# Thieso/BoundPlanner

Hardware: AMD Instinct MI355X
Metric: MPC solves/sec (whole node), iiwa14 7-DOF, N=20 (higher is better)
Workload: dtype f64; 1 GPU; BASELINE configs[2]: 8192-batch, randomized convex-set obstacles, N=20, cold start, tol 1e-5, max_iter 100; a fresh batch every step; batch_per_gpu=8192, horizon=20, distinct_batches=22, fresh_batches=16, hess=2, solver_handles_in_flight=4, batches_in_flight=44, pool_slots=16384

## Files before the change

__graft_entry__.py:

```python
import os
import subprocess
import sys

ROOT = os.path.dirname(os.path.abspath(__file__))
CSRC = os.path.join(ROOT, "boundplanner_amd", "csrc")
HIP_LIB = os.path.join(CSRC, "libboundmpc_hip.so")
_COMMON = ["bmpc_platform_hip.hpp", "bmpc_device.hpp", "bmpc_internal.hpp"]
_HANDLE = ["bmpc_handle.hpp", "bmpc_pipeline.hpp", "bmpc_stage.hpp", "bmpc_robot.hpp", "../../include/boundmpc.h"]
HIP_OBJS = {
    "bmpc_fk.o": ("bmpc_fk.hip", [], _COMMON),
    "bmpc_pipeline.o": ("bmpc_pipeline.hip", [], _COMMON + ["bmpc_pipeline.hpp", "bmpc_pair_kernels.hpp", "bmpc_ric_kernel.hpp",
                                                            "bmpc_stage.hpp", "bmpc_stage_matrix.hpp"]),
    "bmpc_loop.o": ("bmpc_loop.hip", [], _COMMON + ["bmpc_loop.hpp", "bmpc_freespace.hpp", "bmpc_robot.hpp", "../../include/boundmpc.h"]),
    "bmpc_capi.o": ("bmpc_capi.hip", [], _COMMON + _HANDLE + ["bmpc_staging.hpp"]),
    "bmpc_capi_batch.o": ("bmpc_capi_batch.hip", [], _COMMON + _HANDLE + ["bmpc_staging.hpp", "bmpc_ik.hpp", "bmpc_sets.hpp",
                                                                          "bmpc_freespace.hpp"]),
    "bmpc_ik.o": ("bmpc_ik.hip", [], _COMMON + ["bmpc_ik.hpp"]),
    "bmpc_sets.o": ("bmpc_sets.hip", [], _COMMON + ["bmpc_sets.hpp", "bmpc_freespace.hpp"]),
}


def _stale(target, deps):
    if not os.path.exists(target):
        return True
    t = os.path.getmtime(target)
    return any(os.path.getmtime(d) > t for d in deps if os.path.exists(d))


def build():
    flags = ["--offload-arch=gfx950", "-O3", "-std=c++17", "-fPIC", "-ffp-contract=on"]
    objs, relink = [], not os.path.exists(HIP_LIB)
    for obj, (src, defs, hdrs) in HIP_OBJS.items():
        o = os.path.join(CSRC, obj)
        if _stale(o, [os.path.join(CSRC, f) for f in [src] + hdrs]):
            subprocess.check_call(["hipcc", *flags, *defs, "-c", os.path.join(CSRC, src), "-o", o])
        objs.append(o)
    if relink or _stale(HIP_LIB, objs):
        subprocess.check_call(["hipcc", "--offload-arch=gfx950", "-shared", "-fPIC", "-o", HIP_LIB, *objs])
    subprocess.check_call(["make", "-C", os.path.join(ROOT, "oracle")], stdout=subprocess.DEVNULL)
    sys.path.insert(0, ROOT)
    import boundplanner_amd
    from boundplanner_amd import solver
    lib = solver.load_library()
    for name in solver.EXPORTS:
        getattr(lib, name)


def smoke():
    sys.path.insert(0, ROOT)
    sys.path.insert(0, os.path.join(ROOT, "tests"))
    import numpy as np
    import oracle_lib as O
    from boundplanner_amd import scenes
    from boundplanner_amd.solver import HipBoundMPC
    N, B = 10, 8
    be = HipBoundMPC(N)
    batch = scenes.make_batch(B, N, 1024, be.fk)
    r = be.solve_batch(batch["x0"], batch["lbx"], batch["ubx"], batch["p"])
    ro = O.solve_batch(N, batch["x0"], batch["lbx"], batch["ubx"], batch["p"])
    assert (r["status"] == 0).all(), r["status"]
    err = np.abs(r["x"][:, 28 * N:40 * N] - ro["x"][:, 28 * N:40 * N]).max()
    assert err < 2e-5, err
    print(f"smoke ok: B={B} N={N} iters={r['iters'].tolist()} max|pv_hip - pv_oracle|={err:.2e} kernel {be.last_kernel_ms():.2f} ms")


if __name__ == "__main__":
    build()
    if len(sys.argv) > 1 and sys.argv[1] == "smoke":
        smoke()
```

boundplanner_amd/csrc/bmpc_internal.hpp:

```cpp
#pragma once
#include <hip/hip_runtime.h>

#include <cstddef>
#include <cstdlib>

struct bmpc_handle;
namespace bmpc {
struct RobotConst;
struct IkOpts;
struct SetScene;
template <int DEV> struct PipeArgsT;
typedef PipeArgsT<0> PipeArgsH;
}

inline int env_int(const char* name, int dflt) { const char* e = getenv(name); return e ? atoi(e) : dflt; }

extern "C" {
hipError_t bmpc_launch_fk(int B, const bmpc::RobotConst* rc, const double* q, const double* dq, double* ee_pos, double* ee_rot,
                          double* col_pts, double* jac, double* dvdq, hipStream_t st);
hipError_t bmpc_launch_spin(int ms, hipStream_t st);
hipError_t bmpc_launch_ik(int B, int log2s, const bmpc::IkOpts* o, const bmpc::RobotConst* rc, const double* pd, const double* rd,
                          const double* q0, const double* lo, const double* hi, double* q, double* cost, double* pos_err,
                          double* rot_err, int* iters, int* status, int* seed, hipStream_t st);
hipError_t bmpc_launch_sets(int B, int segment, int fixed_mid, int optimize, const bmpc::SetScene* sc, double* AAt_ws,
                            const double* p0, const double* p1, double* A, double* b, int* nrows, double* q, double* c, int* rounds,
                            int* newton, int* collision, int* status, hipStream_t st);
hipError_t bmpc_launch_sets_parts(int B, int mode, const bmpc::SetScene* sc, const double* E, const double* p, const double* A_in,
                                  const double* b_in, const int* m_in, double* A, double* b, int* nrows, double* q, double* c,
                                  int* newton, int* status, hipStream_t st);
hipError_t bmpc_pipe_launch_init(const bmpc::PipeArgsH* A, int n0, hipStream_t st);
hipError_t bmpc_pipe_launch_retire_out(const bmpc::PipeArgsH* A, int n_max, hipStream_t st);
hipError_t bmpc_pipe_launch_retire_admit(const bmpc::PipeArgsH* A, int n_max, int refill, hipStream_t st);
hipError_t bmpc_pipe_launch_step(bmpc::PipeArgsH* A, int n_act, hipStream_t st, hipEvent_t e0, hipEvent_t e1, int* was_lat);
hipError_t bmpc_pipe_launch_mult(const bmpc::PipeArgsH* A, hipStream_t st);
hipError_t bmpc_pipe_launch_stage_matrices(const bmpc::PipeArgsH* A, const double* d_t, const double* d_z, const double* d_lam_pi,
                                           double* d_H, hipStream_t st);
hipError_t bmpc_pipe_launch_newton_step(bmpc::PipeArgsH* A, const double* d_t, const double* d_z, const int* d_mode, double* d_dzeta,
                                        double* d_dt, double* d_dz, double* d_state, hipStream_t st);
hipError_t bmpc_pipe_launch_line_search(bmpc::PipeArgsH* A, const double* d_t, const double* d_z, const int* d_mode,
                                        const double* d_plant0, const double* d_plant1, double* d_dzeta, double* d_dt, double* d_dz,
                                        double* d_state, double* d_zeta0, double* d_t0, double* d_z0, double* d_zeta1, double* d_t1,
                                        double* d_z1, double* d_ls, hipStream_t st, const double* d_ctl_plant = nullptr,
                                        double* d_ctl = nullptr);
void bmpc_pipe_ls_sizes(int* plant0, int* plant1, int* out);
void bmpc_pipe_ctl_sizes(int* plant, int* out);
void bmpc_pipe_build_table(int* tbl);
size_t bmpc_pipe_state_bytes(void);

void bmpc_handle_retain(bmpc_handle* h);
void bmpc_handle_release(bmpc_handle* h);
typedef int (*bmpc_retire_hook)(void* ctx, const int* d_done, const int* d_n_done, int n_max, void* stream);
int bmpc_solve_dev_hooked(bmpc_handle* h, int B, const double* d_x0, const double* d_lbx, const double* d_ubx, const double* d_p,
                          double* d_x, double* d_f, int* d_iters, int* d_status, double* d_viol, void* stream, bmpc_retire_hook hook,
                          void* hook_ctx, const int* d_cont);
}
```

boundplanner_amd/csrc/bmpc_pair_kernels.hpp:

```cpp
#pragma once
#include "bmpc_pipeline.hpp"

namespace bmpc {

BMPC_INL constexpr int sym7(int i, int j) { return i <= j ? (i * 7 - i * (i - 1) / 2 + (j - i)) : (j * 7 - j * (j - 1) / 2 + (i - j)); }
BMPC_INL constexpr int sym3(int i, int j) { return i <= j ? (i * 3 - i * (i - 1) / 2 + (j - i)) : (j * 3 - j * (j - 1) / 2 + (i - j)); }

struct StagePoint {
    double zeta[NZ], y[NZ];
    KinT K;
    double Jl[3][7];
    SegCtx C;
};

BMPC_INL void load_zeta(GCD arr, size_t NP, size_t pi, double* z) {
    BMPC_UNROLL
    for (int i = 0; i < NZ; i++) z[i] = arr[(size_t)i * NP + pi];
}

BMPC_INL void stage_point(const PipeArgs& A, PGP pg, const double* iw0, int k, const DynC dc, StagePoint& S) {
    nat_all(S.zeta, dc, S.y);
    kin_chain(A.rc, S.y + Z_Q, S.K);
    kin_jlin(S.K, S.Jl);
    kin_vel(S.K, S.Jl, S.y + Z_DQ, S.C.v);
    BMPC_UNROLL
    for (int a = 0; a < 3; a++) { S.C.pose[a] = S.K.pee[a]; S.C.pose[3 + a] = S.y[Z_PI + a] + 0.5 * dc.dt * S.C.v[3 + a]; }
    seg_ctx_eval(pg, A.N, k, S.y, iw0, S.C);
}

BMPC_INL void defect_all(const double* z, const double* zn, const double* vang, const DynC d, double* r) {
    BMPC_UNROLL
    for (int i = 0; i < 7; i++) {
        r[Z_Q + i] = z[Z_Q + i] + d.dt * z[Z_DQ + i] + 0.5 * d.dt * d.dt * z[Z_DDQ + i] + d.b3 * z[Z_U + i] - zn[Z_Q + i];
        r[Z_DQ + i] = z[Z_DQ + i] + d.dt * z[Z_DDQ + i] + d.b2 * z[Z_U + i] - zn[Z_DQ + i];
        r[Z_DDQ + i] = z[Z_DDQ + i] + d.b1 * z[Z_U + i] - zn[Z_DDQ + i];
    }
    BMPC_UNROLL
    for (int a = 0; a < 3; a++) r[Z_PI + a] = z[Z_PI + a] + d.dt * vang[a] - zn[Z_PI + a];
    r[Z_RS] = z[Z_RS] + d.dt * z[Z_DRS] - zn[Z_RS];
    r[Z_PS] = z[Z_PS] + d.dt * z[Z_DPS] - zn[Z_PS];
    BMPC_UNROLL
    for (int i = 0; i < 6; i++) r[Z_D + i] = z[Z_D + i] - zn[Z_D + i];
}

struct InitVisitor {
    const PipeArgs* A; size_t pi; bool valid;
    double th, ls;
    BMPC_INL void set(int s, double h) {
        double t = fmax(-h, 1e-2);
        th += fabs(h + t); ls += log(t);
        if (!valid) return;
        size_t o = (size_t)s * A->NP + pi;
        A->t[o] = t; A->t_t[o] = t; A->z[o] = 1.0; A->z_t[o] = 1.0;
    }
    BMPC_INL void skip(int s) {
        if (!valid) return;
        size_t o = (size_t)s * A->NP + pi;
        A->t[o] = 1.0; A->t_t[o] = 1.0; A->z[o] = 0.0; A->z_t[o] = 0.0;
    }
    BMPC_INL void diag(int s, int, double, double h) { set(s, h); }
    BMPC_INL void zdiag(int s, int, double, double h) { set(s, h); }
    BMPC_INL void pose(int s, const double*, int, double h) { set(s, h); }
    template <int S0, int CNT> BMPC_INL void group(unsigned) {}
    template <int C> BMPC_INL void point_begin(unsigned) {}
    template <int C> BMPC_INL void point(int s, const double*, double h) { set(s, h); }
    template <int C> BMPC_INL void point_end() {}
};

BMPC_KBODY void k_init_body(const PipeArgs& A, int wave, int lane, LDSD* lds_par) {
    const int count = A.L.cnt[9], N = A.N;
    if (wave * ipw_of(N) >= count) return;
    PairMap m = pair_map(A, A.L.admit, count, wave, lane);
    const int k = m.k, n_w = 44 * N + 6;
    const DynC dc = make_dync(A.o.dt);
    const size_t row = (size_t)A.src[m.b];
    GCD x0 = A.x0 + row * n_w;
    GCD lbx = A.lbx + row * n_w;
    GCD ubx = A.ubx + row * n_w;
    PGP pg = stage_params(A, A.L.admit, count, wave, lane, m, lds_par);
    double iw0[3];
    BMPC_UNROLL
    for (int c = 0; c < 3; c++) iw0[c] = lbx[28 * N + (3 + c) * N];
    StagePoint S;
    BMPC_UNROLL
    for (int j = 0; j < 7; j++) {
        double uu = x0[21 * N + j * N + k];
        S.zeta[Z_Q + j] = x0[j * N + k] - dc.c3 * uu;
        S.zeta[Z_DQ + j] = x0[7 * N + j * N + k] - dc.c2 * uu;
        S.zeta[Z_DDQ + j] = x0[14 * N + j * N + k] - dc.c1 * uu;
        S.zeta[Z_U + j] = uu;
    }
    double prot[3];
    BMPC_UNROLL
    for (int c = 0; c < 3; c++) { prot[c] = x0[28 * N + (3 + c) * N + k]; S.zeta[Z_PI + c] = prot[c]; }
    {
        double rs = x0[40 * N + 6 + k], drs = x0[41 * N + 6 + k], ps = x0[42 * N + 6 + k], dps = x0[43 * N + 6 + k];
        S.zeta[Z_RS] = rs - dc.dt / 2 * drs; S.zeta[Z_PS] = ps - dc.dt / 2 * dps;
        S.zeta[Z_DRS] = drs; S.zeta[Z_DPS] = dps;
    }
    BMPC_UNROLL
    for (int i = 0; i < 6; i++) S.zeta[Z_D + i] = x0[40 * N + i];
    nat_all(S.zeta, dc, S.y);
    kin_chain(A.rc, S.y + Z_Q, S.K);
    BMPC_UNROLL
    for (int a = 0; a < 3; a++) {
        double w = 0;
        BMPC_UNROLL
        for (int j = 0; j < 7; j++) w += S.K.zx[j][a] * S.y[Z_DQ + j];
        S.zeta[Z_PI + a] = prot[a] - dc.dt / 2 * w;
    }
    stage_point(A, pg, iw0, k, dc, S);
    if (m.valid)
        BMPC_UNROLL
        for (int i = 0; i < NZ; i++) { A.zeta[(size_t)i * A.NP + m.pi] = S.zeta[i]; A.zeta_t[(size_t)i * A.NP + m.pi] = S.zeta[i]; }
    InitVisitor v{&A, m.pi, m.valid, 0.0, 0.0};
    walk_rows(pg, lbx, ubx, N, k, S.y, S.zeta, S.K, S.C, v);
    if (m.valid)
        for (int s = S_END; s < NSLOT; s++) v.skip(s);
    double th = v.th;
    if (k < N - 1) {
        double zn[NX];
        BMPC_UNROLL
        for (int j = 0; j < 7; j++) {
            double uu = x0[21 * N + j * N + k + 1];
            zn[Z_Q + j] = x0[j * N + k + 1] - dc.c3 * uu;
            zn[Z_DQ + j] = x0[7 * N + j * N + k + 1] - dc.c2 * uu;
            zn[Z_DDQ + j] = x0[14 * N + j * N + k + 1] - dc.c1 * uu;
        }
        {
            double yq[7], ydq[7];
            BMPC_UNROLL
            for (int j = 0; j < 7; j++) { double uu = x0[21 * N + j * N + k + 1]; yq[j] = zn[Z_Q + j] + dc.c3 * uu; ydq[j] = zn[Z_DQ + j] + dc.c2 * uu; }
            KinT Kn;
            kin_chain(A.rc, yq, Kn);
            BMPC_UNROLL
            for (int a = 0; a < 3; a++) {
                double w = 0;
                BMPC_UNROLL
                for (int j = 0; j < 7; j++) w += Kn.zx[j][a] * ydq[j];
                zn[Z_PI + a] = x0[28 * N + (3 + a) * N + k + 1] - dc.dt / 2 * w;
            }
        }
        zn[Z_RS] = x0[40 * N + 6 + k + 1] - dc.dt / 2 * x0[41 * N + 6 + k + 1];
        zn[Z_PS] = x0[42 * N + 6 + k + 1] - dc.dt / 2 * x0[43 * N + 6 + k + 1];
        BMPC_UNROLL
        for (int i = 0; i < 6; i++) zn[Z_D + i] = x0[40 * N + i];
        double rdef[NX];
        defect_all(S.zeta, zn, S.C.v + 3, dc, rdef);
        BMPC_UNROLL
        for (int i = 0; i < NX; i++) th += fabs(rdef[i]);
    }
    if (k == 1) {
        double x1fix[24];
        x1fix_eval(lbx, N, dc.dt, x1fix);
        BMPC_UNROLL
        for (int i = 0; i < 24; i++) th += fabs(x1fix[i] - S.zeta[i]);
    }
    if (m.valid) {
        GD P = A.part + m.pi;
        P[PT_F1 * A.NP] = S.C.fv; P[PT_TH1 * A.NP] = th; P[PT_LS1 * A.NP] = v.ls;
    }
}

struct RowAcc {
    const PipeArgs* A; size_t pi; bool valid; double ad;
    GCD tc, zc;
    double cmax, csum, cmin, zsum, prim, nrows;
    BMPC_INL void init(const PipeArgs* A_, size_t pi_, bool valid_, double ad_, GCD tc_, GCD zc_) {
        A = A_; pi = pi_; valid = valid_; ad = ad_; tc = tc_; zc = zc_;
        cmax = 0; csum = 0; cmin = 1e300; zsum = 0; prim = 0; nrows = 0;
    }
    BMPC_INL void row(int s, double h, double& sg, double& r0, double& r1, double& zz) {
        size_t o = (size_t)s * A->NP + pi;
        row_tz(tc[o], zc[o], h, sg, r0, r1, zz);
    }
    BMPC_INL void row_tz(double t, double z_in, double h, double& sg, double& r0, double& r1, double& zz) {
        zz = z_in;
        r1 = BMPC_RCP(t); sg = zz * r1; r0 = sg * (h + t);
        double c = t * zz;
        cmax = fmax(cmax, c); csum += c; cmin = fmin(cmin, c); zsum += zz;
        prim = fmax(prim, fabs(h + t));
        nrows += 1.0;
    }
};

template <int S0_, int CNT_> struct RowPre {
    static constexpr int S0 = S0_, CNT = CNT_;
    double t[CNT_], z[CNT_];
    BMPC_INL void load(const PipeArgs& A, GCD tc, GCD zc, size_t pi) {
        BMPC_UNROLL
        for (int i = 0; i < CNT_; i++) { size_t o = (size_t)(S0_ + i) * A.NP + pi; t[i] = tc[o]; z[i] = zc[o]; }
    }
};
template <int I0_, int CNT_> struct BndPre {
    static constexpr int I0 = I0_, CNT = CNT_;
    double ub[CNT_], lb[CNT_];
    BMPC_INL void load(GCD lbx, GCD ubx, int N, int k) {
        BMPC_UNROLL
        for (int i = 0; i < CNT_; i++) {
            const int I = I0_ + i, blk = I / 7, jj = I % 7;
            size_t wi = (size_t)blk * 7 * N + (size_t)jj * N + k;
            ub[i] = ubx[wi]; lb[i] = lbx[wi];
        }
    }
};

struct PointAsm {
    RowAcc* R; const KinT* K;
    double M3[6], mc[3], sc, b30[3], b31[3], b3z[3], bc0, bc1, bcz;
    double Hqq[28], gq0[7], gq1[7], gqz[7], dD[6], gD0[6], gD1[6], gDz[6], cd[6][7], Fc[6][3];
    double pt[15], pz[15];
    BMPC_INL void init() {
        BMPC_UNROLL
        for (int i = 0; i < 28; i++) Hqq[i] = 0;
        BMPC_UNROLL
        for (int i = 0; i < 7; i++) { gq0[i] = 0; gq1[i] = 0; gqz[i] = 0; }
    }
    BMPC_INL void skip(int) {}
    template <int C> BMPC_INL void point_begin(unsigned act) {
        BMPC_UNROLL
        for (int i = 0; i < 15; i++) {
            size_t o = (size_t)(S_COL + 15 * C + i) * R->A->NP + R->pi;
            if ((act >> i) & 1u) { pt[i] = R->tc[o]; pz[i] = R->zc[o]; } else { pt[i] = 1.0; pz[i] = 0.0; }
        }
        BMPC_UNROLL
        for (int i = 0; i < 6; i++) M3[i] = 0;
        BMPC_UNROLL
        for (int i = 0; i < 3; i++) { mc[i] = 0; b30[i] = 0; b31[i] = 0; b3z[i] = 0; }
        sc = 0; bc0 = 0; bc1 = 0; bcz = 0;
    }
    template <int C> BMPC_INL void point(int s, const double* a, double h) {
        double sg, r0, r1, zz;
        R->row_tz(pt[s - (S_COL + 15 * C)], pz[s - (S_COL + 15 * C)], h, sg, r0, r1, zz);
        BMPC_UNROLL
        for (int i = 0; i < 3; i++) {
            BMPC_UNROLL
            for (int j = i; j < 3; j++) M3[sym3(i, j)] += sg * a[i] * a[j];
            mc[i] -= sg * a[i]; b30[i] += r0 * a[i]; b31[i] += r1 * a[i]; b3z[i] += zz * a[i];
        }
        sc += sg; bc0 -= r0; bc1 -= r1; bcz -= zz;
    }
    template <int C> BMPC_INL void point_end() {
        constexpr int nj = PointNJ<C>::value;
        const double* pc = kin_point<C>(*K);
        double Jp[nj][3], T[nj][3];
        BMPC_UNROLL
        for (int i = 0; i < nj; i++) {
            double r[3] = {pc[0] - K->o[i][0], pc[1] - K->o[i][1], pc[2] - K->o[i][2]};
            cross3r(K->zx[i], r, Jp[i]);
            BMPC_UNROLL
            for (int a = 0; a < 3; a++) T[i][a] = M3[sym3(a, 0)] * Jp[i][0] + M3[sym3(a, 1)] * Jp[i][1] + M3[sym3(a, 2)] * Jp[i][2];
        }
        BMPC_UNROLL
        for (int i = 0; i < nj; i++) {
            BMPC_UNROLL
            for (int j = i; j < nj; j++) Hqq[sym7(i, j)] += Jp[i][0] * T[j][0] + Jp[i][1] * T[j][1] + Jp[i][2] * T[j][2];
            gq0[i] += Jp[i][0] * b30[0] + Jp[i][1] * b30[1] + Jp[i][2] * b30[2];
            gq1[i] += Jp[i][0] * b31[0] + Jp[i][1] * b31[1] + Jp[i][2] * b31[2];
            gqz[i] += Jp[i][0] * b3z[0] + Jp[i][1] * b3z[1] + Jp[i][2] * b3z[2];
        }
        BMPC_UNROLL
        for (int i = 0; i < 7; i++) {
            double v = (i < nj) ? (Jp[i < nj ? i : 0][0] * mc[0] + Jp[i < nj ? i : 0][1] * mc[1] + Jp[i < nj ? i : 0][2] * mc[2]) : 0.0;
            cd[C][i] = v;
        }
        dD[C] = sc; gD0[C] = bc0; gD1[C] = bc1; gDz[C] = bcz;
        BMPC_UNROLL
        for (int a = 0; a < 3; a++) Fc[C][a] = b3z[a];
    }
};

struct PointRes {
    GCD base; size_t NP;
    double cd5_[7], gq_[21], hqq_[28], dD_[6], gD_[18];
    BMPC_INL double at(int slot) const { return base[(size_t)slot * NP]; }
    BMPC_INL void load_p17() {
        BMPC_UNROLL
        for (int i = 0; i < 7; i++) cd5_[i] = at(SD_CD5 + i);
        BMPC_UNROLL
        for (int i = 0; i < 21; i++) gq_[i] = at(SD_GQ + i);
    }
    BMPC_INL void load_hqq() {
        BMPC_UNROLL
        for (int i = 0; i < 28; i++) hqq_[i] = at(SD_HQQ + i);
    }
    BMPC_INL void load_dg() {
        BMPC_UNROLL
        for (int i = 0; i < 6; i++) dD_[i] = at(SD_DD + i);
        BMPC_UNROLL
        for (int i = 0; i < 18; i++) gD_[i] = at(SD_GD + i);
    }
    BMPC_INL double cd5(int i) const { return cd5_[i]; }
    BMPC_INL double hqq(int e) const { return hqq_[e]; }
    BMPC_INL double gq(int v, int i) const { return gq_[7 * v + i]; }
    BMPC_INL double dD(int c) const { return dD_[c]; }
    BMPC_INL double gD(int v, int c) const { return gD_[6 * v + c]; }
};

struct PoseAsm {
    RowAcc* R;
    double M6[21], mS[3][6], sS[3], bp0[6], bp1[6], bpz[6], bS0[3], bS1[3], bSz[3];
    BMPC_INL void init(const double* Hp, const double* g12) {
        BMPC_UNROLL
        for (int i = 0; i < 21; i++) M6[i] = Hp[i];
        BMPC_UNROLL
        for (int s = 0; s < 3; s++) {
            sS[s] = 0; bS0[s] = 0; bS1[s] = 0; bSz[s] = 0;
            BMPC_UNROLL
            for (int i = 0; i < 6; i++) mS[s][i] = 0;
        }
        BMPC_UNROLL
        for (int i = 0; i < 6; i++) { bp0[i] = g12[i]; bpz[i] = g12[i]; bp1[i] = 0; }
    }
    template <int NA, int SEL> BMPC_INL void add(const double* a, double h, double t, double z) {
        double sg, r0, r1, zz;
        R->row_tz(t, z, h, sg, r0, r1, zz);
        BMPC_UNROLL
        for (int i = 0; i < NA; i++) {
            BMPC_UNROLL
            for (int j = i; j < NA; j++) M6[sym6(i, j)] += sg * a[i] * a[j];
            bp0[i] += r0 * a[i]; bp1[i] += r1 * a[i]; bpz[i] += zz * a[i];
            if (SEL > 0) mS[SEL > 0 ? SEL - 1 : 0][i] -= sg * a[i];
        }
        if (SEL > 0) { sS[SEL - 1] += sg; bS0[SEL - 1] -= r0; bS1[SEL - 1] -= r1; bSz[SEL - 1] -= zz; }
    }
};

template <class V, class G1>
BMPC_INL void walk_pose_rows(PGP pg, int N, int k, const double* y, const SegCtx& C, V& v, const G1& g1, double t_phi, double z_phi) {
    static_assert(G1::S0 == S_EE && G1::CNT == 21, "pose row group");
    {
        PGP a = pg + P_ASET + 45 * C.s;
        BMPC_UNROLL
        for (int rr = 0; rr < 15; rr++) {
            double a3[3] = {a[rr], a[rr + 15], a[rr + 30]};
            double bb = pg[P_BSET + rr * 4 + C.s];
            if (!(a3[0] == 0 && a3[1] == 0 && a3[2] == 0 && bb > 0))
                v.template add<3, 1>(a3, a3[0] * C.pose[0] + a3[1] * C.pose[1] + a3[2] * C.pose[2] - bb - y[Z_PS], g1.t[rr], g1.z[rr]);
        }
    }
    BMPC_UNROLL
    for (int m = 0; m < 3; m++) {
        double al[6];
        BMPC_UNROLL
        for (int c = 0; c < 6; c++) al[c] = -C.gs[m][c];
        v.template add<6, 2>(C.gs[m], C.proj[m] - C.ub[m] - y[Z_RS], g1.t[S_ROTU - S_EE + m], g1.z[S_ROTU - S_EE + m]);
        v.template add<6, 2>(al, -(C.proj[m] - C.lb[m] + y[Z_RS]), g1.t[S_ROTL - S_EE + m], g1.z[S_ROTL - S_EE + m]);
    }
    v.template add<3, 0>(C.dpp, C.phi - (C.phiend + 0.005), t_phi, z_phi);
}
template <class V, class G2>
BMPC_INL void walk_pose_rows_term(PGP pg, int N, int k, const double* y, const SegCtx& C, V& v, const G2& g2) {
    static_assert(G2::S0 == S_TSET && G2::CNT == 21, "terminal pose row group");
    const bool term = (k == N - 1);
    if (term) {
        PGP a = pg + P_ASET + 45 * C.n;
        BMPC_UNROLL
        for (int rr = 0; rr < 15; rr++) {
            double an[3] = {a[rr], a[rr + 15], a[rr + 30]};
            double bn = pg[P_BSET + rr * 4 + C.n];
            if (!(an[0] == 0 && an[1] == 0 && an[2] == 0 && bn + pg[P_SLACKS0 + 5] > 0)) {
                double a1 = dot3(an, C.bp1), a2 = dot3(an, C.bp2);
                double bnew = bn - dot3(an, C.pend);
                double a3[3];
                BMPC_UNROLL
                for (int c = 0; c < 3; c++) {
                    double tt = 0;
                    BMPC_UNROLL
                    for (int a_ = 0; a_ < 3; a_++) tt += (a1 * C.bp1[a_] + a2 * C.bp2[a_]) * C.Dep[a_][c];
                    a3[c] = tt;
                }
                v.template add<3, 3>(a3, a1 * C.tz[0] + a2 * C.tz[1] - bnew - C.sl[5], g2.t[rr], g2.z[rr]);
            }
        }
        BMPC_UNROLL
        for (int m = 0; m < 3; m++) {
            double al[6];
            BMPC_UNROLL
            for (int c = 0; c < 6; c++) al[c] = -C.gsn[m][c];
            v.template add<6, 3>(C.gsn[m], C.projn[m] - C.ubn[m] - C.sl[5], g2.t[S_TROTU - S_TSET + m], g2.z[S_TROTU - S_TSET + m]);
            v.template add<6, 3>(al, -(C.projn[m] - C.lbn[m] + C.sl[5]), g2.t[S_TROTL - S_TSET + m], g2.z[S_TROTL - S_TSET + m]);
        }
    }
}

template <int I, class V, class RP, class BP>
BMPC_INL void walk_diag_pos(const RP& rp, const BP& bp, int k, const double* y, V& v) {
    if constexpr (I < 28) {
        constexpr int blk = I / 7, jj = I % 7;
        constexpr int pos = (blk == 0 ? Z_Q : blk == 1 ? Z_DQ : blk == 2 ? Z_DDQ : Z_U) + jj;
        static_assert(I >= BP::I0 && I < BP::I0 + BP::CNT && 2 * I >= RP::S0 && 2 * I + 1 < RP::S0 + RP::CNT, "preloaded range");
        const double ub = bp.ub[I - BP::I0], lb = bp.lb[I - BP::I0];
        if (ub < BIGB) v.diag(1.0, y[pos] - ub, rp.t[2 * I - RP::S0], rp.z[2 * I - RP::S0]);
        if (lb > -BIGB) v.diag(-1.0, lb - y[pos], rp.t[2 * I + 1 - RP::S0], rp.z[2 * I + 1 - RP::S0]);
    } else if constexpr (I < 32) {
        constexpr int pos = (I == 28 ? Z_RS : I == 29 ? Z_DRS : I == 30 ? Z_PS : Z_DPS);
        constexpr int s = S_NONNEG + (I == 28 ? 0 : I == 29 ? 1 : I == 30 ? 2 : 3);
        static_assert(s >= RP::S0 && s < RP::S0 + RP::CNT, "preloaded range");
        v.diag(-1.0, -y[pos], rp.t[s - RP::S0], rp.z[s - RP::S0]);
    } else if constexpr (I < 38) {
        constexpr int s = S_D1 + (I - 32);
        static_assert(s >= RP::S0 && s < RP::S0 + RP::CNT, "preloaded range");
        if (k == 1) v.diag(-1.0, -y[Z_D + I - 32], rp.t[s - RP::S0], rp.z[s - RP::S0]);
    }
}

struct DiagAsm {
    RowAcc* R;
    double D, g0, g1, gz;
    BMPC_INL void begin() { D = 0; g0 = 0; g1 = 0; gz = 0; }
    BMPC_INL void diag(double coef, double h, double t, double z) {
        double sg, r0, r1, zz;
        R->row_tz(t, z, h, sg, r0, r1, zz);
        D += sg; g0 += coef * r0; g1 += coef * r1; gz += coef * zz;
    }
};

template <int J>
BMPC_INL void chain_cols(const KinT& K, const double Jl[3][7], const double G[6][7], double hdt, double* cO, double* cV) {
    if constexpr (J < 7) {
        BMPC_UNROLL
        for (int a = 0; a < 3; a++) { cO[a] = Jl[a][J]; cO[3 + a] = hdt * G[3 + a][J]; cV[a] = G[a][J]; cV[3 + a] = G[3 + a][J]; }
    } else if constexpr (J < 14) {
        BMPC_UNROLL
        for (int a = 0; a < 3; a++) { cO[a] = 0; cO[3 + a] = hdt * K.zx[J - 7][a]; cV[a] = Jl[a][J - 7]; cV[3 + a] = K.zx[J - 7][a]; }
    } else {
        BMPC_UNROLL
        for (int a = 0; a < 6; a++) { cO[a] = (a == 3 + (J - 14)) ? 1.0 : 0.0; cV[a] = 0; }
    }
}

struct ChainOut { double g17[3][17]; };

template <int J, int I, class EM>
BMPC_INL void chain_rows(const KinT& K, const double Jl[3][7], const double G[6][7], double hdt, const double* t1,
                         const double* t2, const PointRes& PR, EM& E) {
    if constexpr (I <= J) {
        double cO[6], cV[6];
        chain_cols<I>(K, Jl, G, hdt, cO, cV);
        double s = 0;
        BMPC_UNROLL
        for (int a = 0; a < 6; a++) s += cO[a] * t1[a] + cV[a] * t2[a];
        if constexpr (J < 7) s += PR.hqq(sym7(I, J));
        E.put(s);
        chain_rows<J, I + 1>(K, Jl, G, hdt, t1, t2, PR, E);
    }
}
template <int J, class EM>
BMPC_INL void chain_column(const KinT& K, const double Jl[3][7], const double G[6][7], double hdt, const double* M6,
                           const double* Hv, const PointRes& PR, EM& E) {
    double cO[6], cV[6], t1[6], t2[6];
    chain_cols<J>(K, Jl, G, hdt, cO, cV);
    BMPC_UNROLL
    for (int a = 0; a < 6; a++) {
        double s1 = 0, s2 = 0;
        BMPC_UNROLL
        for (int b = 0; b < 6; b++) { s1 += M6[sym6(a, b)] * cO[b]; s2 += Hv[sym6(a, b)] * cV[b]; }
        t1[a] = s1; t2[a] = s2;
    }
    chain_rows<J, 0>(K, Jl, G, hdt, t1, t2, PR, E);
}
template <int J, class EM>
BMPC_INL void chain_all(const KinT& K, const double Jl[3][7], const double G[6][7], double hdt, const double* M6,
                        const double* Hv, const PointRes& PR, EM& E) {
    if constexpr (J < 17) {
        chain_column<J>(K, Jl, G, hdt, M6, Hv, PR, E);
        chain_all<J + 1>(K, Jl, G, hdt, M6, Hv, PR, E);
    }
}
template <int I, int IEND, class RP, class BP, class EM>
BMPC_INL void p17_emit_all(const PipeArgs& A, PGP pg, const RP& rp, const BP& bp, int k, const double* y, const KinT& K,
                           const double Jl[3][7], const double G[6][7], double hdt, RowAcc& R, const PointRes& PA,
                           const PoseAsm& P, const double* bv, EM& E) {
    if constexpr (I < IEND) {
        PGP wts = pg + P_W;
        double cO[6], cV[6];
        chain_cols<I>(K, Jl, G, hdt, cO, cV);
        BMPC_UNROLL
        for (int sl = 0; sl < 3; sl++) {
            double s = 0;
            BMPC_UNROLL
            for (int a = 0; a < 6; a++) s += cO[a] * P.mS[sl][a];
            if (sl == 2 && I < 7) s += PA.cd5(I < 7 ? I : 0);
            E.put(s);
        }
        double g0 = 0, g1 = 0, gz = 0;
        BMPC_UNROLL
        for (int a = 0; a < 6; a++) {
            g0 += cO[a] * P.bp0[a] + cV[a] * bv[a];
            g1 += cO[a] * P.bp1[a];
            gz += cO[a] * P.bpz[a] + cV[a] * bv[a];
        }
        constexpr int DI = I < 14 ? I : 38 + (I - 14);
        DiagAsm dgv;
        dgv.R = &R;
        dgv.begin();
        if constexpr (DI < 38) walk_diag_pos<DI>(rp, bp, k, y, dgv);
        double D = dgv.D;
        g0 += dgv.g0; g1 += dgv.g1; gz += dgv.gz;
        if constexpr (I < 7) { g0 += PA.gq(0, I); g1 += PA.gq(1, I); gz += PA.gq(2, I); }
        if constexpr (I >= 7 + 2 && I <= 7 + 4) {
            const double w2 = 2 * wts[6], val = w2 * y[Z_DQ + I - 7];
            D += w2; g0 += val; gz += val;
        }
        E.put(D); E.put(g0); E.put(g1); E.put(gz);
        p17_emit_all<I + 1, IEND>(A, pg, rp, bp, k, y, K, Jl, G, hdt, R, PA, P, bv, E);
    }
}

template <class EM>
BMPC_INL void curvature_emit(const KinT& K, const double Jl[3][7], const double* dq, const double* Fp, const double* Fv,
                             const double Fc[6][3], const double* sa, const double* sbq, const double* sbdq, double sc1, EM& E) {
    const int njc[6] = {2, 3, 4, 5, 6, 4};
    double tri[28];
    BMPC_UNROLL
    for (int bq = 6; bq >= 0; bq--) {
        double zx[7][3], Jc[3][7];
        BMPC_UNROLL
        for (int i = 0; i < 7; i++)
            BMPC_UNROLL
            for (int x = 0; x < 3; x++) { zx[i][x] = K.zx[i][x]; Jc[x][i] = Jl[x][i]; BMPC_PIN(zx[i][x]); BMPC_PIN(Jc[x][i]); }
        BMPC_UNROLL
        for (int a = 0; a <= bq; a++) {
            const int m = a < bq ? a : bq, M = a < bq ? bq : a;
            double cM[3] = {Jc[0][M], Jc[1][M], Jc[2][M]}, zc[3];
            cross3r(zx[m], cM, zc);
            double acc = dot3(Fp, zc);
            BMPC_UNROLL
            for (int c = 0; c < 6; c++)
                if (M < njc[c]) {
                    const double* pc = (c < 5) ? K.o[c + 2] : K.pl4;
                    double r[3] = {pc[0] - K.o[M][0], pc[1] - K.o[M][1], pc[2] - K.o[M][2]}, cc[3];
                    cross3r(zx[M], r, cc);
                    cross3r(zx[m], cc, zc);
                    acc += dot3(Fc[c], zc);
                }
            BMPC_UNROLL
            for (int j = 0; j < 7; j++) {
                const int m1 = a < j ? a : j, M1 = a < j ? j : a;
                double c1[3] = {Jc[0][M1], Jc[1][M1], Jc[2][M1]};
                double t1[3] = {0, 0, 0}, t2[3], dzm[3], dcM[3];
                if (bq < m1) { cross3r(zx[bq], zx[m1], dzm); cross3r(dzm, c1, t1); }
                const int m2 = bq < M1 ? bq : M1, M2 = bq < M1 ? M1 : bq;
                double c2[3] = {Jc[0][M2], Jc[1][M2], Jc[2][M2]};
                cross3r(zx[m2], c2, dcM);
                cross3r(zx[m1], dcM, t2);
                double lin = Fv[0] * (t1[0] + t2[0]) + Fv[1] * (t1[1] + t2[1]) + Fv[2] * (t1[2] + t2[2]);
                double ang = 0;
                if (a < j) {
                    double u1[3] = {0, 0, 0}, u2[3] = {0, 0, 0}, tmp[3];
                    if (bq < a) { cross3r(zx[bq], zx[a], tmp); cross3r(tmp, zx[j], u1); }
                    if (bq < j) { cross3r(zx[bq], zx[j], tmp); cross3r(zx[a], tmp, u2); }
                    ang = Fv[3] * (u1[0] + u2[0]) + Fv[4] * (u1[1] + u2[1]) + Fv[5] * (u1[2] + u2[2]);
                }
                acc += dq[j] * (lin + ang);
            }
            tri[sym7(a, bq)] = acc + (sc1 * sa[a] * sa[bq] + sbq[a] * sa[bq] + sa[a] * sbq[bq]);
            BMPC_PIN(tri[sym7(a, bq)]);
        }
    }
    BMPC_UNROLL
    for (int a = 0; a < 7; a++)
        BMPC_UNROLL
        for (int bq = 0; bq < 7; bq++) E.put(tri[sym7(a, bq)]);
    BMPC_UNROLL
    for (int i = 0; i < 7; i++)
        BMPC_UNROLL
        for (int j = 0; j < 7; j++) {
            const int m = i < j ? i : j, M = i < j ? j : i;
            double cM[3] = {Jl[0][M], Jl[1][M], Jl[2][M]}, zc[3];
            cross3r(K.zx[m], cM, zc);
            double acc = dot3(Fv, zc);
            if (i < j) { double zz[3]; cross3r(K.zx[i], K.zx[j], zz); acc += dot3(Fv + 3, zz); }
            E.put(acc + sa[i] * sbdq[j]);
        }
}

template <int I, class RP, class BP, class EM>
BMPC_INL void dg_emit_all(const PipeArgs& A, PGP pg, const RP& rp, const BP& bp, int k, bool term,
                          const double* y, RowAcc& R, const PointRes& PA, const PoseAsm& PO, EM& E) {
    if constexpr (I < 38) {
        PGP wts = pg + P_W;
        DiagAsm dgv;
        dgv.R = &R;
        dgv.begin();
        walk_diag_pos<I>(rp, bp, k, y, dgv);
        double D = dgv.D, g0 = dgv.g0, g1 = dgv.g1, gz = dgv.gz;
        if constexpr (I == 30) { D += PO.sS[0]; g0 += PO.bS0[0]; g1 += PO.bS1[0]; gz += PO.bSz[0]; }
        if constexpr (I == 28) { D += PO.sS[1]; g0 += PO.bS0[1]; g1 += PO.bS1[1]; gz += PO.bSz[1]; }
        if constexpr (I >= 32 && I < 38) {
            constexpr int c = I - 32;
            D += PA.dD(c); g0 += PA.gD(0, c); g1 += PA.gD(1, c); gz += PA.gD(2, c);
            if constexpr (c == 5) { D += PO.sS[2]; g0 += PO.bS0[2]; g1 += PO.bS1[2]; gz += PO.bSz[2]; }
        }
        {
            double w2 = 0, extra = 0;
            bool has = false;
            if constexpr (I >= 21 && I < 28) { w2 = 2 * wts[7]; has = true; }
            else if constexpr (I == 28 || I == 30) { w2 = 2 * wts[9]; has = true; }
            else if constexpr (I == 29 || I == 31) { w2 = 2 * wts[10]; has = true; }
            else if constexpr (I >= 32 && I < 38) {
                constexpr int i = I - 32;
                w2 = term ? (2 * wts[10] + (i != 4 ? 2 * wts[8] : 0.0)) : 0.0;
                extra = (term && i != 4) ? 2 * wts[8] * pg[P_SLACKS0 + i] : 0.0;
                has = true;
            }
            if (has) {
                double val = w2 * y[dg_pos_c(I)] + extra;
                D += w2; g0 += val; gz += val;
            }
        }
        E.put(D); E.put(g0); E.put(g1); E.put(gz);
        dg_emit_all<I + 1>(A, pg, rp, bp, k, term, y, R, PA, PO, E);
    }
}

BMPC_KBODY void k_pose_body(const PipeArgs& A, int wave, int lane, LDSD* lds_par) {
    const int count = A.L.cnt[0], N = A.N;
    if (wave * ipw_of(N) >= count) return;
    PairMap m = pair_map(A, A.L.eval, count, wave, lane);
    const int k = m.k, n_w = 44 * N + 6;
    const bool term = (k == N - 1);
    const DynC dc = make_dync(A.o.dt);
    GCD lbx = A.lbx + (size_t)A.src[m.b] * n_w;
    PGP pg = stage_params(A, A.L.eval, count, wave, lane, m, lds_par);
    double iw0[3];
    BMPC_UNROLL
    for (int c = 0; c < 3; c++) iw0[c] = lbx[28 * N + (3 + c) * N];
    StagePoint S;
    const int flip = A.st[m.b].flip;
    GCD zc = cur_zeta(A, flip), tc = cur_t(A, flip), zcur = cur_z(A, flip);
    load_zeta(zc, A.NP, m.pi, S.zeta);
    RowPre<S_EE, 21> rp_pose;
    rp_pose.load(A, tc, zcur, m.pi);
    const double t_phi = tc[(size_t)S_PHI * A.NP + m.pi], z_phi = zcur[(size_t)S_PHI * A.NP + m.pi];
    nat_all(S.zeta, dc, S.y);
    kin_chain(A.rc, S.y + Z_Q, S.K);
    kin_jlin(S.K, S.Jl);
    kin_vel(S.K, S.Jl, S.y + Z_DQ, S.C.v);
    BMPC_UNROLL
    for (int a = 0; a < 3; a++) { S.C.pose[a] = S.K.pee[a]; S.C.pose[3 + a] = S.y[Z_PI + a] + 0.5 * dc.dt * S.C.v[3 + a]; }
    BMPC_UNROLL
    for (int a = 0; a < 6; a++) { BMPC_PIN(S.C.pose[a]); BMPC_PIN(S.C.v[a]); }
    seg_ctx_eval(pg, A.N, k, S.y, iw0, S.C);
    double g12[12], Hp[21];
    cost_grad12(pg, S.C, term, g12);
    {
        double HvX[21];
        cost_hess(pg, S.C, term, Hp, HvX);
    }
    if (m.valid && A.o.hess == 2) {
        GD Sg = A.part + (size_t)PT_SIG * A.NP + m.pi;
        const double c2 = 2 * S.C.sig * S.C.dsig;
        Sg[0] = 2 * S.C.sig * (60.0 * S.C.dsig * (1.0 - 2.0 * S.C.sig)) * S.C.er2ep2;
        BMPC_UNROLL
        for (int a = 0; a < 3; a++) Sg[(size_t)(1 + a) * A.NP] = S.C.dpp[a];
        BMPC_UNROLL
        for (int bb = 0; bb < 6; bb++) {
            double ge = S.C.Der[0][bb] * S.C.er[0] + S.C.Der[1][bb] * S.C.er[1] + S.C.Der[2][bb] * S.C.er[2];
            if (bb < 3) ge += S.C.Dep[0][bb] * S.C.ep[0] + S.C.Dep[1][bb] * S.C.ep[1] + S.C.Dep[2][bb] * S.C.ep[2];
            Sg[(size_t)(4 + bb) * A.NP] = c2 * ge;
        }
    }
    RowAcc R;
    R.init(&A, m.pi, m.valid, 0.0, tc, zcur);
    PoseAsm PO;
    PO.R = &R;
    PO.init(Hp, g12);
    walk_pose_rows(pg, N, k, S.y, S.C, PO, rp_pose, t_phi, z_phi);
    {
        RowPre<S_TSET, 21> rp_term;
        rp_term.load(A, tc, zcur, m.pi);
        walk_pose_rows_term(pg, N, k, S.y, S.C, PO, rp_term);
    }
    if (!m.valid) return;
    const double hdt = 0.5 * dc.dt;
    if (A.o.hess == 2) {
        GD F = A.part + (size_t)PT_FORCE * A.NP + m.pi;
        BMPC_UNROLL
        for (int a = 0; a < 3; a++) F[(size_t)a * A.NP] = PO.bpz[a];
        BMPC_UNROLL
        for (int a = 0; a < 6; a++) F[(size_t)(3 + a) * A.NP] = g12[6 + a] + (a >= 3 ? hdt * PO.bpz[a] : 0.0);
    }
    GD Pz = A.part + (size_t)PT_POSE * A.NP + m.pi;
    BMPC_UNROLL
    for (int i = 0; i < 21; i++) Pz[(size_t)(PZ_M6 + i) * A.NP] = PO.M6[i];
    BMPC_UNROLL
    for (int sl = 0; sl < 3; sl++) {
        BMPC_UNROLL
        for (int i = 0; i < 6; i++) Pz[(size_t)(PZ_MS + 6 * sl + i) * A.NP] = PO.mS[sl][i];
        Pz[(size_t)(PZ_SS + sl) * A.NP] = PO.sS[sl];
        Pz[(size_t)(PZ_BS0 + sl) * A.NP] = PO.bS0[sl]; Pz[(size_t)(PZ_BS1 + sl) * A.NP] = PO.bS1[sl]; Pz[(size_t)(PZ_BSZ + sl) * A.NP] = PO.bSz[sl];
    }
    BMPC_UNROLL
    for (int i = 0; i < 6; i++) {
        Pz[(size_t)(PZ_BP0 + i) * A.NP] = PO.bp0[i]; Pz[(size_t)(PZ_BP1 + i) * A.NP] = PO.bp1[i]; Pz[(size_t)(PZ_BPZ + i) * A.NP] = PO.bpz[i];
        Pz[(size_t)(PZ_BV + i) * A.NP] = g12[6 + i];
    }
    Pz[(size_t)(PZ_KKT + 0) * A.NP] = R.cmax; Pz[(size_t)(PZ_KKT + 1) * A.NP] = R.csum; Pz[(size_t)(PZ_KKT + 2) * A.NP] = R.cmin;
    Pz[(size_t)(PZ_KKT + 3) * A.NP] = R.zsum; Pz[(size_t)(PZ_KKT + 4) * A.NP] = R.prim; Pz[(size_t)(PZ_KKT + 5) * A.NP] = R.nrows;
    BMPC_UNROLL
    for (int a = 0; a < 3; a++) Pz[(size_t)(PZ_VANG + a) * A.NP] = S.C.v[3 + a];
}

template <int MODE>
BMPC_KBODY void k_eval_body(const PipeArgs& A, int wave, int lane, LDSD* lds) {
    const int count = A.L.cnt[0], N = A.N;
    if (wave * ipw_of(N) >= count) return;
    PairMap m = pair_map(A, A.L.eval, count, wave, lane);
    const int k = m.k, n_w = 44 * N + 6;
    const bool term = (k == N - 1);
    const DynC dc = make_dync(A.o.dt);
    GCD lbx = A.lbx + (size_t)A.src[m.b] * n_w;
    GCD ubx = A.ubx + (size_t)A.src[m.b] * n_w;
    PGP pg = stage_params(A, A.L.eval, count, wave, lane, m, lds + EM_DOUBLES + 8);
    if constexpr (MODE == 2) {
        struct { double zeta[NZ], y[NZ]; KinT K; double Jl[3][7]; } S;
        const int flip = A.st[m.b].flip;
        load_zeta(cur_zeta(A, flip), A.NP, m.pi, S.zeta);
        nat_all(S.zeta, dc, S.y);
        kin_chain(A.rc, S.y + Z_Q, S.K);
        kin_jlin(S.K, S.Jl);
        double G[6][7];
        kin_G(S.K, S.Jl, S.y + Z_DQ, G);
        PointRes PA;
        PA.base = A.part + (size_t)PT_SIDE * A.NP + m.pi; PA.NP = A.NP;
        GCD Pz = A.part + (size_t)PT_POSE * A.NP + m.pi;
        double Hv[21], M6[21];
        cost_hess_v(pg, N, k, Hv);
        BMPC_UNROLL
        for (int i = 0; i < 21; i++) M6[i] = Pz[(size_t)(PZ_M6 + i) * A.NP];
        PA.load_hqq();
        DirectEmitter D;
        D.out = A.hrec + hrec_of(A, m.b, m.k) + F_H17; D.valid = m.valid; D.f = 0;
        chain_all<0>(S.K, S.Jl, G, 0.5 * dc.dt, M6, Hv, PA, D);
        return;
    }
    const double ad = A.st[m.b].ad;
    EmitterT<MODE == 1> E;
    E.init(lds, A.hrec, lane, hrec_of(A, m.b, m.k), m.valid, 0, F_H17, F_EW);
    BMPC_SYNC();
    struct { double zeta[NZ], y[NZ]; KinT K; double Jl[3][7]; } S;
    const int flip = A.st[m.b].flip;
    GCD zc = cur_zeta(A, flip), tc = cur_t(A, flip), zcur = cur_z(A, flip);
    load_zeta(zc, A.NP, m.pi, S.zeta);
    nat_all(S.zeta, dc, S.y);
    kin_chain(A.rc, S.y + Z_Q, S.K);
    kin_jlin(S.K, S.Jl);
    double G[6][7];
    kin_G(S.K, S.Jl, S.y + Z_DQ, G);
    RowAcc R;
    R.init(&A, m.pi, m.valid, ad, tc, zcur);
    PoseAsm PO;
    PO.R = &R;
    GCD Pz = A.part + (size_t)PT_POSE * A.NP + m.pi;
    {
        GCD Sd = A.part + (size_t)(PT_SIDE + SD_KKT) * A.NP + m.pi;
        R.cmax = fmax(Sd[0], Pz[(size_t)(PZ_KKT + 0) * A.NP]); R.csum = Sd[A.NP] + Pz[(size_t)(PZ_KKT + 1) * A.NP];
        R.cmin = fmin(Sd[2 * A.NP], Pz[(size_t)(PZ_KKT + 2) * A.NP]); R.zsum = Sd[3 * A.NP] + Pz[(size_t)(PZ_KKT + 3) * A.NP];
        R.prim = fmax(Sd[4 * A.NP], Pz[(size_t)(PZ_KKT + 4) * A.NP]); R.nrows = Sd[5 * A.NP] + Pz[(size_t)(PZ_KKT + 5) * A.NP];
    }
    PointRes PA;
    PA.base = A.part + (size_t)PT_SIDE * A.NP + m.pi; PA.NP = A.NP;
    {
        double cdv[35];
        BMPC_UNROLL
        for (int i = 0; i < 35; i++) cdv[i] = PA.at(SD_CD + i);
        BMPC_UNROLL
        for (int i = 0; i < 35; i++) E.put(cdv[i]);
    }
    const double hdt = 0.5 * dc.dt;
    {
        double bvv[6];
        BMPC_UNROLL
        for (int sl = 0; sl < 3; sl++)
            BMPC_UNROLL
            for (int i = 0; i < 6; i++) PO.mS[sl][i] = Pz[(size_t)(PZ_MS + 6 * sl + i) * A.NP];
        BMPC_UNROLL
        for (int i = 0; i < 6; i++) {
            PO.bp0[i] = Pz[(size_t)(PZ_BP0 + i) * A.NP]; PO.bp1[i] = Pz[(size_t)(PZ_BP1 + i) * A.NP]; PO.bpz[i] = Pz[(size_t)(PZ_BPZ + i) * A.NP];
            bvv[i] = Pz[(size_t)(PZ_BV + i) * A.NP];
        }
        PA.load_p17();
        {
            RowPre<0, 14> rp_a;
            BndPre<0, 7> bp_a;
            rp_a.load(A, tc, zcur, m.pi); bp_a.load(lbx, ubx, N, k);
            p17_emit_all<0, 7>(A, pg, rp_a, bp_a, k, S.y, S.K, S.Jl, G, hdt, R, PA, PO, bvv, E);
        }
            {
            RowPre<14, 14> rp_a;
            BndPre<7, 7> bp_a;
            rp_a.load(A, tc, zcur, m.pi); bp_a.load(lbx, ubx, N, k);
            p17_emit_all<7, 17>(A, pg, rp_a, bp_a, k, S.y, S.K, S.Jl, G, hdt, R, PA, PO, bvv, E);
        }
    }
    if constexpr (MODE == 1) {
        BMPC_UNROLL
        for (int i = 0; i < F_EW - F_H17; i++) E.put(0.0);
    } else {
        double Hv[21];
        cost_hess_v(pg, N, k, Hv);
        BMPC_UNROLL
        for (int i = 0; i < 21; i++) PO.M6[i] = Pz[(size_t)(PZ_M6 + i) * A.NP];
        PA.load_hqq();
        BMPC_UNROLL
        for (int a = 0; a < 3; a++)
            BMPC_UNROLL
            for (int j = 0; j < 7; j++) { BMPC_PIN(S.Jl[a][j]); BMPC_PIN(S.K.zx[j][a]); }
        BMPC_UNROLL
        for (int a = 0; a < 6; a++)
            BMPC_UNROLL
            for (int j = 0; j < 7; j++) BMPC_PIN(G[a][j]);
        BMPC_UNROLL
        for (int i = 0; i < 21; i++) BMPC_PIN(PO.M6[i]);
        chain_all<0>(S.K, S.Jl, G, hdt, PO.M6, Hv, PA, E);
    }
    BMPC_UNROLL
    for (int a = 0; a < 3; a++)
        BMPC_UNROLL
        for (int j = 0; j < 7; j++) E.put(G[3 + a][j]);
    BMPC_UNROLL
    for (int a = 0; a < 3; a++)
        BMPC_UNROLL
        for (int j = 0; j < 7; j++) E.put(S.K.zx[j][a]);
    {
        double sz[3] = {0, 0, 0}, sufz[7][3];
        BMPC_UNROLL
        for (int j = 6; j >= 0; j--)
            BMPC_UNROLL
            for (int a = 0; a < 3; a++) { sz[a] += S.K.zx[j][a] * S.y[Z_DQ + j]; sufz[j][a] = sz[a]; }
        BMPC_UNROLL
        for (int mm = 1; mm < 8; mm++)
            BMPC_UNROLL
            for (int a = 0; a < 3; a++) E.put(mm < 7 ? sufz[mm < 7 ? mm : 0][a] : 0.0);
    }
    double zeta2[NZ], y2[NZ];
    load_zeta(zc, A.NP, m.pi, zeta2);
    nat_all(zeta2, dc, y2);
    RowPre<28, 40> rp_b;
    BndPre<14, 14> bp_b;
    rp_b.load(A, tc, zcur, m.pi); bp_b.load(lbx, ubx, N, k);
    BMPC_UNROLL
    for (int sl = 0; sl < 3; sl++) {
        PO.sS[sl] = Pz[(size_t)(PZ_SS + sl) * A.NP];
        PO.bS0[sl] = Pz[(size_t)(PZ_BS0 + sl) * A.NP]; PO.bS1[sl] = Pz[(size_t)(PZ_BS1 + sl) * A.NP]; PO.bSz[sl] = Pz[(size_t)(PZ_BSZ + sl) * A.NP];
    }
    PA.load_dg();
    dg_emit_all<14>(A, pg, rp_b, bp_b, k, term, y2, R, PA, PO, E);
    {
        double sg2[2] = {0, 0}, r2[3][2] = {{0, 0}, {0, 0}, {0, 0}};
        if (k == 1) {
            BMPC_UNROLL
            for (int i = 0; i < 2; i++) {
                double sg, r0, r1, zz;
                R.row_tz(rp_b.t[S_RS1 - 28 + i], rp_b.z[S_RS1 - 28 + i], -zeta2[i ? Z_PS : Z_RS], sg, r0, r1, zz);
                sg2[i] = sg; r2[0][i] = r0; r2[1][i] = r1; r2[2][i] = zz;
            }
        }
        E.put(sg2[0]); E.put(sg2[1]);
        BMPC_UNROLL
        for (int v = 0; v < 3; v++) { E.put(r2[v][0]); E.put(r2[v][1]); }
    }
    double prim = R.prim;
    {
        double rdef[NX];
        if (!term) {
            double zn[NX];
            BMPC_UNROLL
            for (int i = 0; i < NX; i++) zn[i] = zc[(size_t)i * A.NP + m.pi + 1];
            double vang[3];
            BMPC_UNROLL
            for (int a = 0; a < 3; a++) vang[a] = Pz[(size_t)(PZ_VANG + a) * A.NP];
            defect_all(zeta2, zn, vang, dc, rdef);
            BMPC_UNROLL
            for (int i = 0; i < NX; i++) prim = fmax(prim, fabs(rdef[i]));
        } else {
            BMPC_UNROLL
            for (int i = 0; i < NX; i++) rdef[i] = 0;
        }
        BMPC_UNROLL
        for (int i = 0; i < NX; i++) E.put(rdef[i]);
    }
    E.pad_to(512);
    if (k == 1) {
        double x1fix[24];
        x1fix_eval(lbx, N, dc.dt, x1fix);
        BMPC_UNROLL
        for (int i = 0; i < 24; i++) prim = fmax(prim, fabs(x1fix[i] - zeta2[i]));
    }
    if (m.valid) {
        GD P = A.part + m.pi;
        P[PT_CMAX * A.NP] = R.cmax; P[PT_CSUM * A.NP] = R.csum; P[PT_CMIN * A.NP] = R.cmin; P[PT_ZSUM * A.NP] = R.zsum;
        P[PT_PRIM * A.NP] = prim; P[PT_NROWS * A.NP] = R.nrows;
    }
}

BMPC_KBODY void k_points_body(const PipeArgs& A, int wave, int lane, LDSD* lds_par) {
    const int count = A.L.cnt[0], N = A.N;
    if (wave * ipw_of(N) >= count) return;
    PairMap m = pair_map(A, A.L.eval, count, wave, lane);
    if (m.valid && m.k == 1 && A.o.hess == 2 && A.st[m.b].hess_mode) {
        int pos = BMPC_ATOMIC_INC(A.L.cnt + 10);
        A.L.curv[pos] = m.b;
    }
    const DynC dc = make_dync(A.o.dt);
    PGP pg = stage_params(A, A.L.eval, count, wave, lane, m, lds_par);
    double zeta[NZ], y[NZ];
    const int flip = A.st[m.b].flip;
    load_zeta(cur_zeta(A, flip), A.NP, m.pi, zeta);
    nat_all(zeta, dc, y);
    KinT K;
    kin_chain(A.rc, y + Z_Q, K);
    SegCtx C;
    BMPC_UNROLL
    for (int i = 0; i < 6; i++) C.sl[i] = pg[P_SLACKS0 + i] + y[Z_D + i];
    RowAcc R;
    R.init(&A, m.pi, m.valid, 0.0, cur_t(A, flip), cur_z(A, flip));
    PointAsm PA;
    PA.R = &R; PA.K = &K;
    PA.init();
    walk_points<PointAsm, 0>(pg, K, C.sl, PA);
    if (!m.valid) return;
    GD Sd = A.part + (size_t)PT_SIDE * A.NP + m.pi;
    BMPC_UNROLL
    for (int c = 0; c < 5; c++)
        BMPC_UNROLL
        for (int i = 0; i < 7; i++) Sd[(size_t)(SD_CD + 7 * c + i) * A.NP] = PA.cd[c][i];
    BMPC_UNROLL
    for (int i = 0; i < 7; i++) {
        Sd[(size_t)(SD_CD5 + i) * A.NP] = PA.cd[5][i];
        Sd[(size_t)(SD_GQ + i) * A.NP] = PA.gq0[i]; Sd[(size_t)(SD_GQ + 7 + i) * A.NP] = PA.gq1[i]; Sd[(size_t)(SD_GQ + 14 + i) * A.NP] = PA.gqz[i];
    }
    BMPC_UNROLL
    for (int i = 0; i < 28; i++) Sd[(size_t)(SD_HQQ + i) * A.NP] = PA.Hqq[i];
    BMPC_UNROLL
    for (int c = 0; c < 6; c++) {
        Sd[(size_t)(SD_DD + c) * A.NP] = PA.dD[c];
        Sd[(size_t)(SD_GD + c) * A.NP] = PA.gD0[c]; Sd[(size_t)(SD_GD + 6 + c) * A.NP] = PA.gD1[c]; Sd[(size_t)(SD_GD + 12 + c) * A.NP] = PA.gDz[c];
    }
    Sd[(size_t)(SD_KKT + 0) * A.NP] = R.cmax; Sd[(size_t)(SD_KKT + 1) * A.NP] = R.csum; Sd[(size_t)(SD_KKT + 2) * A.NP] = R.cmin;
    Sd[(size_t)(SD_KKT + 3) * A.NP] = R.zsum; Sd[(size_t)(SD_KKT + 4) * A.NP] = R.prim; Sd[(size_t)(SD_KKT + 5) * A.NP] = R.nrows;
    if (A.o.hess == 2) {
        GD F = A.part + (size_t)PT_FORCE * A.NP + m.pi;
        BMPC_UNROLL
        for (int c = 0; c < 6; c++)
            BMPC_UNROLL
            for (int a = 0; a < 3; a++) F[(size_t)(9 + 3 * c + a) * A.NP] = PA.Fc[c][a];
    }
}

BMPC_KBODY void k_curv_body(const PipeArgs& A, int wave, int lane, LDSD* lds) {
    const int count = A.L.cnt[10], N = A.N;
    if (A.o.hess != 2 || wave * ipw_of(N) >= count) return;
    PairMap m = pair_map(A, A.L.curv, count, wave, lane);
    const DynC dc = make_dync(A.o.dt);
    Emitter E;
    E.init(lds, A.hrec, lane, hrec_of(A, m.b, m.k), m.valid, F_CQP);
    BMPC_SYNC();
    double zeta[NZ], y[NZ];
    load_zeta(cur_zeta(A, A.st[m.b].flip), A.NP, m.pi, zeta);
    nat_all(zeta, dc, y);
    KinT K;
    double Jl[3][7];
    kin_chain(A.rc, y + Z_Q, K);
    kin_jlin(K, Jl);
    double Fp[3], Fv[6], Fc[6][3];
    GCD F = A.part + (size_t)PT_FORCE * A.NP + m.pi;
    BMPC_UNROLL
    for (int a = 0; a < 3; a++) Fp[a] = F[(size_t)a * A.NP];
    BMPC_UNROLL
    for (int a = 0; a < 6; a++) Fv[a] = F[(size_t)(3 + a) * A.NP];
    BMPC_UNROLL
    for (int c = 0; c < 6; c++)
        BMPC_UNROLL
        for (int a = 0; a < 3; a++) Fc[c][a] = F[(size_t)(9 + 3 * c + a) * A.NP];
    double sa[7], sbq[7], sbdq[7], sc1;
    {
        GCD Sg = A.part + (size_t)PT_SIG * A.NP + m.pi;
        double dpp[3], gec[6];
        sc1 = Sg[0];
        BMPC_UNROLL
        for (int a = 0; a < 3; a++) dpp[a] = Sg[(size_t)(1 + a) * A.NP];
        BMPC_UNROLL
        for (int a = 0; a < 6; a++) gec[a] = Sg[(size_t)(4 + a) * A.NP];
        double G[6][7];
        kin_G(K, Jl, y + Z_DQ, G);
        const double hdt = 0.5 * dc.dt;
        BMPC_UNROLL
        for (int j = 0; j < 7; j++) {
            sa[j] = dpp[0] * Jl[0][j] + dpp[1] * Jl[1][j] + dpp[2] * Jl[2][j];
            sbq[j] = gec[0] * Jl[0][j] + gec[1] * Jl[1][j] + gec[2] * Jl[2][j]
                     + hdt * (gec[3] * G[3][j] + gec[4] * G[4][j] + gec[5] * G[5][j]);
            sbdq[j] = hdt * (gec[3] * K.zx[j][0] + gec[4] * K.zx[j][1] + gec[5] * K.zx[j][2]);
        }
        BMPC_UNROLL
        for (int i = 0; i < 7; i++)
            BMPC_UNROLL
            for (int a = 0; a < 3; a++) E.put(sa[i] * gec[3 + a]);
    }
    curvature_emit(K, Jl, y + Z_DQ, Fp, Fv, Fc, sa, sbq, sbdq, sc1, E);
    E.pad_to(HREC);
}

BMPC_INL void ls0_instance(const PipeArgs& A, int b) {
    const int N = A.N;
    GST st = A.st + b;
    GCD P = A.part + pair_of(A, b, 1);
    double ap = 1.0, ad = 1.0, dbar = 0, dphif = 0;
    for (int k = 0; k < N - 1; k++) {
        ap = fmin(ap, P[PT_AP * A.NP + k]); ad = fmin(ad, P[PT_AD * A.NP + k]);
        dbar += P[PT_DBAR * A.NP + k]; dphif += P[PT_DPHIF * A.NP + k];
    }
    st->ap = ap; st->ad = ad;
    st->D = dphif + dbar;
    st->phi0 = st->f0 - st->mu * st->ls0;
    if (st->it == 0) { st->theta_max = 1e4 * fmax(1.0, st->th0); st->theta_min = 1e-4 * fmax(1.0, st->th0); }
    if (st->mu != st->filt_mu) { st->nfilt = 0; st->filt_mu = st->mu; }
    st->alpha = (A.o.ls_alpha_mem > 0 && st->it > 0) ? fmin(ap, A.o.ls_alpha_mem * st->alpha) : ap;
    st->bt = 0; st->armijo = 0;
    st->state = ST_TRIAL;
    int pos = BMPC_ATOMIC_INC(A.L.cnt + 2);
    A.L.trial[pos] = b;
}

BMPC_INL bool ls_decide(const PipeArgs& A, int b, double f1, double th1, double ls1, bool requeue) {
    GST st = A.st + b;
    const double mu = st->mu, th0 = st->th0, D = st->D, phi0 = st->phi0, alpha = st->alpha;
    double phi1 = f1 - mu * ls1;
    bool acc = (th1 <= st->theta_max);
    for (int j = 0; acc && j < st->nfilt; j++)
        if (th1 >= st->filt_th[j] && phi1 >= st->filt_phi[j]) acc = false;
    bool armijo_case = false;
    if (acc) {
        bool sw = (th0 <= st->theta_min) && (D < 0) && (alpha * pow(-D, 2.3) > pow(th0, 1.1));
        if (sw) { acc = (phi1 <= phi0 + 1e-4 * alpha * D + 1e-12 * fabs(phi0)); armijo_case = acc; }
        else acc = (th1 <= (1 - 1e-5) * th0) || (phi1 <= phi0 - 1e-5 * th0);
    }
    if (acc || st->bt >= 9) {
        if (!armijo_case) {
            const int MAXF = 8;
            int nf = st->nfilt;
            if (nf == MAXF) { for (int j = 0; j + 1 < MAXF; j++) { st->filt_th[j] = st->filt_th[j + 1]; st->filt_phi[j] = st->filt_phi[j + 1]; } nf--; }
            st->filt_th[nf] = (1 - 1e-5) * th0;
            st->filt_phi[nf] = phi0 - 1e-5 * th0;
            st->nfilt = nf + 1;
        }
        st->f0 = f1; st->th0 = th1; st->ls0 = ls1;
        if (!acc) st->alpha = 1e300;
        st->flip ^= 1;
        st->it += 1;
        int want = (A.o.hess == 2 && (st->err_prev < A.o.hess_switch || (A.o.inertia == 2 && st->stall >= A.o.stall_n))) ? 1 : 0;
        if (A.o.gn_backoff > 0 && want && st->gn_skip > 0) { want = 0; st->gn_skip -= 1; }
        st->hess_mode = want;
        st->state = ST_EVAL;
        int pos = BMPC_ATOMIC_INC(A.L.cnt + 3);
        A.L.eval_next[pos] = b;
        return true;
    }
    st->alpha = 0.5 * alpha; st->bt += 1;
    if (requeue) {
        int pos = BMPC_ATOMIC_INC(A.L.cnt + 4);
        A.L.trial_next[pos] = b;
    }
    return false;
}
BMPC_INL bool ls_instance(const PipeArgs& A, int b, bool requeue) {
    GCD P = A.part + pair_of(A, b, 1);
    double f1 = 0, th1 = 0, ls1 = 0;
    for (int k = 0; k < A.N - 1; k++) { f1 += P[PT_F1 * A.NP + k]; th1 += P[PT_TH1 * A.NP + k]; ls1 += P[PT_LS1 * A.NP + k]; }
    return ls_decide(A, b, f1, th1, ls1, requeue);
}

struct StepVisitor {
    const PipeArgs* A; size_t pi; bool valid;
    double mu, tau;
    const double* dy;
    const double* dzt;
    double dloc[6], dpt[6][3];
    GCD tc, zc;
    double gt[ROW_GROUP_MAX], gz[ROW_GROUP_MAX];
    double rp, rdn, rdd, dbar;
    template <int S0, int CNT> BMPC_INL void group(unsigned act) {
        static_assert(CNT <= ROW_GROUP_MAX, "row group size");
        BMPC_UNROLL
        for (int i = 0; i < CNT; i++) {
            size_t o = (size_t)(S0 + i) * A->NP + pi;
            if ((act >> i) & 1u) { gt[i] = tc[o]; gz[i] = zc[o]; } else { gt[i] = 1.0; gz[i] = 0.0; }
        }
    }
    BMPC_INL void fin(int s, double h, double adot) {
        const double c = -h - adot, t = gt[s - row_group_base(s)], z = gz[s - row_group_base(s)];
        const double rt = BMPC_RCP(t), dti = c - t, dzi = (mu - z * c) * rt;
        if (valid) { size_t o = (size_t)s * A->NP + pi; A->dt[o] = c; }
        rp = fmax(rp, -dti * rt);
        if (-dzi * rdd > rdn * z) { rdn = -dzi; rdd = z; }
        dbar -= mu * dti * rt;
    }
    BMPC_INL void skip(int) {}
    BMPC_INL void diag(int s, int pos, double coef, double h) { fin(s, h, coef * dy[pos]); }
    BMPC_INL void zdiag(int s, int pos, double coef, double h) { fin(s, h, coef * dzt[pos]); }
    BMPC_INL void pose(int s, const double* a, int sel, double h) {
        double adot = 0;
        BMPC_UNROLL
        for (int c = 0; c < 6; c++) adot += a[c] * dloc[c];
        if (sel == 1) adot -= dy[Z_PS];
        else if (sel == 2) adot -= dy[Z_RS];
        else if (sel == 3) adot -= dy[Z_D + 5];
        fin(s, h, adot);
    }
    template <int C> BMPC_INL void point_begin(unsigned act) { group<S_COL + 15 * C, 15>(act); }
    template <int C> BMPC_INL void point(int s, const double* a, double h) {
        fin(s, h, a[0] * dpt[C][0] + a[1] * dpt[C][1] + a[2] * dpt[C][2] - dy[Z_D + C]);
    }
    template <int C> BMPC_INL void point_end() {}
};

template <int C>
BMPC_INL void point_dirs(const KinT& K, const double* dyq, double dpt[6][3]) {
    if constexpr (C < 6) {
        constexpr int nj = PointNJ<C>::value;
        const double* pc = kin_point<C>(K);
        double s[3] = {0, 0, 0};
        BMPC_UNROLL
        for (int i = 0; i < nj; i++) {
            double r[3] = {pc[0] - K.o[i][0], pc[1] - K.o[i][1], pc[2] - K.o[i][2]}, c[3];
            cross3r(K.zx[i], r, c);
            s[0] += c[0] * dyq[i]; s[1] += c[1] * dyq[i]; s[2] += c[2] * dyq[i];
        }
        dpt[C][0] = s[0]; dpt[C][1] = s[1]; dpt[C][2] = s[2];
        point_dirs<C + 1>(K, dyq, dpt);
    }
}

BMPC_KBODY void k_step_body(const PipeArgs& A, int wave, int lane, LDSD* lds_par) {
    const int count = A.L.cnt[1], N = A.N;
    if (wave * ipw_of(N) >= count) return;
    PairMap m = pair_map(A, A.L.step, count, wave, lane);
    const int k = m.k, n_w = 44 * N + 6;
    const bool term = (k == N - 1);
    const DynC dc = make_dync(A.o.dt);
    GCD lbx = A.lbx + (size_t)A.src[m.b] * n_w;
    GCD ubx = A.ubx + (size_t)A.src[m.b] * n_w;
    PGP pg = stage_params(A, A.L.step, count, wave, lane, m, lds_par);
    PGP wts = pg + P_W;
    const double mu = A.st[m.b].mu;
    double iw0[3];
    BMPC_UNROLL
    for (int c = 0; c < 3; c++) iw0[c] = lbx[28 * N + (3 + c) * N];
    StagePoint S;
    const int flip = A.st[m.b].flip;
    load_zeta(cur_zeta(A, flip), A.NP, m.pi, S.zeta);
    double dzt[NZ], dy[NZ];
    load_zeta(A.dz, A.NP, m.pi, dzt);
    nat_all(S.zeta, dc, S.y);
    nat_all(dzt, dc, dy);
    StepVisitor V;
    V.A = &A; V.pi = m.pi; V.valid = m.valid; V.mu = mu; V.tau = fmax(0.99, 1.0 - mu); V.tc = cur_t(A, flip); V.zc = cur_z(A, flip);
    V.dy = dy; V.dzt = dzt; V.rp = 0.0; V.rdn = 0.0; V.rdd = 1.0; V.dbar = 0.0;
    walk_rows<StepVisitor, WR_BOX>(pg, lbx, ubx, N, k, S.y, S.zeta, S.K, S.C, V);
    BMPC_PIN(V.rp); BMPC_PIN(V.rdn); BMPC_PIN(V.rdd); BMPC_PIN(V.dbar);
    BMPC_UNROLL
    for (int j = 0; j < 7; j++) BMPC_PIN(S.y[Z_Q + j]);
    kin_chain(A.rc, S.y + Z_Q, S.K);
    kin_jlin(S.K, S.Jl);
    kin_vel(S.K, S.Jl, S.y + Z_DQ, S.C.v);
    BMPC_UNROLL
    for (int a = 0; a < 3; a++) { S.C.pose[a] = S.K.pee[a]; S.C.pose[3 + a] = S.y[Z_PI + a] + 0.5 * dc.dt * S.C.v[3 + a]; }
    double dv[6];
    {
        double G[6][7];
        kin_G(S.K, S.Jl, S.y + Z_DQ, G);
        BMPC_UNROLL
        for (int a = 0; a < 6; a++) {
            double s = 0;
            BMPC_UNROLL
            for (int j = 0; j < 7; j++) s += G[a][j] * dy[Z_Q + j] + (a < 3 ? S.Jl[a][j] : S.K.zx[j][a - 3]) * dy[Z_DQ + j];
            dv[a] = s;
        }
    }
    BMPC_UNROLL
    for (int a = 0; a < 3; a++) {
        double s = 0;
        BMPC_UNROLL
        for (int j = 0; j < 7; j++) s += S.Jl[a][j] * dy[Z_Q + j];
        V.dloc[a] = s;
        V.dloc[3 + a] = dy[Z_PI + a] + 0.5 * dc.dt * dv[3 + a];
    }
    point_dirs<0>(S.K, dy + Z_Q, V.dpt);
    BMPC_UNROLL
    for (int a = 0; a < 6; a++) { BMPC_PIN(dv[a]); BMPC_PIN(V.dloc[a]); BMPC_PIN(S.C.pose[a]); BMPC_PIN(S.C.v[a]); }
    BMPC_UNROLL
    for (int c = 0; c < 6; c++)
        BMPC_UNROLL
        for (int a = 0; a < 3; a++) BMPC_PIN(V.dpt[c][a]);
    seg_ctx_eval(pg, A.N, k, S.y, iw0, S.C);
    double g12[12];
    cost_grad12(pg, S.C, term, g12);
    double dphi_f = 0;
    BMPC_UNROLL
    for (int a = 0; a < 6; a++) dphi_f += g12[a] * V.dloc[a] + g12[6 + a] * dv[a];
    BMPC_UNROLL
    for (int j = 2; j <= 4; j++) dphi_f += 2 * wts[6] * S.y[Z_DQ + j] * dy[Z_DQ + j];
    BMPC_UNROLL
    for (int j = 0; j < 7; j++) dphi_f += 2 * wts[7] * S.y[Z_U + j] * dy[Z_U + j];
    dphi_f += 2 * wts[9] * S.y[Z_RS] * dy[Z_RS] + 2 * wts[10] * S.y[Z_DRS] * dy[Z_DRS] +
              2 * wts[9] * S.y[Z_PS] * dy[Z_PS] + 2 * wts[10] * S.y[Z_DPS] * dy[Z_DPS];
    if (term)
        BMPC_UNROLL
        for (int i = 0; i < 6; i++) {
            double gg = 2 * wts[10] * S.y[Z_D + i] + (i != 4 ? 2 * wts[8] * (pg[P_SLACKS0 + i] + S.y[Z_D + i]) : 0.0);
            dphi_f += gg * dy[Z_D + i];
        }
    walk_rows<StepVisitor, WR_POSE>(pg, lbx, ubx, N, k, S.y, S.zeta, S.K, S.C, V);
    BMPC_PIN(V.rp); BMPC_PIN(V.rdn); BMPC_PIN(V.rdd); BMPC_PIN(V.dbar);
    walk_rows<StepVisitor, WR_PT0 | WR_PT1>(pg, lbx, ubx, N, k, S.y, S.zeta, S.K, S.C, V);
    if (m.valid) {
        GD P = A.part + m.pi;
        P[PT_DPHIF * A.NP] = dphi_f;
        P[PT_AP * A.NP] = (V.rp > 0) ? V.tau / V.rp : 1.0; P[PT_AD * A.NP] = (V.rdn > 0) ? V.tau / (V.rdn / V.rdd) : 1.0; P[PT_DBAR * A.NP] = V.dbar;
    }
    BMPC_FENCE_SYNC();
    if (m.valid && m.k == 1) ls0_instance(A, m.b);
}

struct TrialVisitor {
    const PipeArgs* A; size_t pi; bool valid;
    double alpha;
    GCD tc; GD tn_out;
    bool dual; double ad, mu; GCD zc; GD zn_out;
    double gt[ROW_GROUP_MAX], gc[ROW_GROUP_MAX];
    double thr;
    double lp; int le;
    template <int S0, int CNT> BMPC_INL void group(unsigned act) {
        static_assert(CNT <= ROW_GROUP_MAX, "row group size");
        double gz[CNT];
        BMPC_UNROLL
        for (int i = 0; i < CNT; i++) {
            size_t o = (size_t)(S0 + i) * A->NP + pi;
            if ((act >> i) & 1u) { gt[i] = tc[o]; gc[i] = A->dt[o]; gz[i] = zc[o]; } else { gt[i] = 1.0; gc[i] = 1.0; gz[i] = 0.0; }
        }
        if (dual) {
            BMPC_UNROLL
            for (int i = 0; i < CNT; i++)
                if (gz[i] > 0.0) zn_out[(size_t)(S0 + i) * A->NP + pi] = gz[i] + ad * ((mu - gz[i] * gc[i]) * BMPC_RCP(gt[i]));
        }
    }
    BMPC_INL void fin(int s, double h) {
        const double t = gt[s - row_group_base(s)];
        double tn = t + alpha * (gc[s - row_group_base(s)] - t);
        if (A->o.slack_reset) tn = fmax(tn, -h);
        thr += fabs(h + tn);
        int e;
        lp = frexp(lp * tn, &e); le += e;
        if (valid) tn_out[(size_t)s * A->NP + pi] = tn;
    }
    BMPC_INL void skip(int) {}
    BMPC_INL void diag(int s, int, double, double h) { fin(s, h); }
    BMPC_INL void zdiag(int s, int, double, double h) { fin(s, h); }
    BMPC_INL void pose(int s, const double*, int, double h) { fin(s, h); }
    template <int C> BMPC_INL void point_begin(unsigned act) { group<S_COL + 15 * C, 15>(act); }
    template <int C> BMPC_INL void point(int s, const double*, double h) { fin(s, h); }
    template <int C> BMPC_INL void point_end() {}
};

struct TrialPart { double f, th, thr, lp; int le; };
template <int ROLES>
BMPC_INL void trial_part(const PipeArgs& A, PGP pg, int b, int k, size_t pi, bool live, bool dual, double alpha, int flip, TrialPart& R,
                         GD t_out = nullptr, GD zeta_out = nullptr) {
    const int N = A.N, n_w = 44 * N + 6;
    const bool term = (k == N - 1);
    const DynC dc = make_dync(A.o.dt);
    GCD lbx = A.lbx + (size_t)A.src[b] * n_w;
    GCD ubx = A.ubx + (size_t)A.src[b] * n_w;
    GCD zc = cur_zeta(A, flip);
    StagePoint S;
    BMPC_UNROLL
    for (int i = 0; i < NZ; i++) S.zeta[i] = zc[(size_t)i * A.NP + pi] + alpha * A.dz[(size_t)i * A.NP + pi];
    if constexpr ((ROLES & WR_POSE) != 0) {
        GD zo = zeta_out ? zeta_out : oth_zeta(A, flip);
        if (live)
            BMPC_UNROLL
            for (int i = 0; i < NZ; i++) zo[(size_t)i * A.NP + pi] = S.zeta[i];
    }
    nat_all(S.zeta, dc, S.y);
    TrialVisitor V;
    V.A = &A; V.pi = pi; V.valid = live; V.alpha = alpha; V.thr = 0.0; V.lp = 1.0; V.le = 0; V.tc = cur_t(A, flip); V.tn_out = t_out ? t_out : oth_t(A, flip);
    V.dual = dual; V.ad = A.st[b].ad; V.mu = A.st[b].mu; V.zc = cur_z(A, flip); V.zn_out = oth_z(A, flip);
    if constexpr ((ROLES & WR_BOX) != 0) walk_rows<TrialVisitor, WR_BOX>(pg, lbx, ubx, N, k, S.y, S.zeta, S.K, S.C, V);
    BMPC_SCHED_FENCE();
    if constexpr ((ROLES & (WR_POSE | WR_PT0 | WR_PT1)) != 0) kin_chain(A.rc, S.y + Z_Q, S.K);
    R.th = 0.0; R.f = 0.0;
    if constexpr ((ROLES & WR_POSE) != 0) {
        double iw0[3];
        BMPC_UNROLL
        for (int c = 0; c < 3; c++) iw0[c] = lbx[28 * N + (3 + c) * N];
        kin_jlin(S.K, S.Jl);
        kin_vel(S.K, S.Jl, S.y + Z_DQ, S.C.v);
        double th = 0;
        if (!term) {
            double zn[NX], rdef[NX];
            BMPC_UNROLL
            for (int i = 0; i < NX; i++) zn[i] = zc[(size_t)i * A.NP + pi + 1] + alpha * A.dz[(size_t)i * A.NP + pi + 1];
            defect_all(S.zeta, zn, S.C.v + 3, dc, rdef);
            BMPC_UNROLL
            for (int i = 0; i < NX; i++) th += fabs(rdef[i]);
        }
        if (k == 1) {
            double x1fix[24];
            x1fix_eval(lbx, N, dc.dt, x1fix);
            BMPC_UNROLL
            for (int i = 0; i < 24; i++) th += fabs(x1fix[i] - S.zeta[i]);
        }
        BMPC_SCHED_FENCE();
        BMPC_UNROLL
        for (int a = 0; a < 3; a++) { S.C.pose[a] = S.K.pee[a]; S.C.pose[3 + a] = S.y[Z_PI + a] + 0.5 * dc.dt * S.C.v[3 + a]; }
        seg_ctx_eval(pg, A.N, k, S.y, iw0, S.C);
        walk_rows<TrialVisitor, WR_POSE>(pg, lbx, ubx, N, k, S.y, S.zeta, S.K, S.C, V);
        R.th = th; R.f = S.C.fv;
    }
    BMPC_SCHED_FENCE();
    if constexpr ((ROLES & (WR_PT0 | WR_PT1)) != 0) walk_rows<TrialVisitor, ROLES & (WR_PT0 | WR_PT1)>(pg, lbx, ubx, N, k, S.y, S.zeta, S.K, S.C, V);
    R.thr = V.thr; R.lp = V.lp; R.le = V.le;
}

template <int NW>
BMPC_KBODY void k_trial_body_t(const PipeArgs& A, int wave, int tid, LDSD* lds_par) {
    static_assert(NW == 1 || NW == 4, "parts of the trial walk");
    const int count = A.L.cnt[2], N = A.N;
    if (wave * ipw_of(N) >= count) return;
    const int lane = tid & 63, role = tid >> 6;
    const PairMap m = pair_map(A, A.L.trial, count, wave, lane);
    const int ipw = ipw_of(N);
    (void)stage_params<true, 64 * NW>(A, A.L.trial, count, wave, tid, m, lds_par);
    LDSD* ended = lds_par + (size_t)ipw * NPARL;
    LDSD* comb = ended + IPW_MAX;
    if (tid < IPW_MAX) ended[tid] = (tid < ipw && wave * ipw + tid < count) ? 0.0 : 1.0;
    BMPC_SYNC();
    const int flip = A.st[m.b].flip;
    for (int round = 0;; round++) {
        int b = m.b, k = m.k, li = m.li;
        BMPC_OPAQUE_I(b); BMPC_OPAQUE_I(k); BMPC_OPAQUE_I(li);
        const size_t pi = pair_of(A, b, k);
        PGP pg = lds_par + li * NPARL;
        const bool live = m.valid && ended[li] == 0.0;
        const double alpha = live ? A.st[b].alpha : 0.0;
        TrialPart R;
        if constexpr (NW == 1) trial_part<WR_ALL>(A, pg, b, k, pi, live, live && round == 0, alpha, flip, R);
        else {
            TrialPart Q;
            if (role == 0) trial_part<WR_POSE>(A, pg, b, k, pi, live, live && round == 0, alpha, flip, Q);
            else if (role == 1) trial_part<WR_BOX>(A, pg, b, k, pi, live, live && round == 0, alpha, flip, Q);
            else if (role == 2) trial_part<WR_PT0>(A, pg, b, k, pi, live, live && round == 0, alpha, flip, Q);
            else trial_part<WR_PT1>(A, pg, b, k, pi, live, live && round == 0, alpha, flip, Q);
            LDSD* c = comb + (size_t)(role * 64 + lane) * TRIAL_COMB;
            c[0] = Q.thr; c[1] = Q.lp; c[2] = (double)Q.le;
            if (role == 0) { c[3] = Q.th; c[4] = Q.f; }
            BMPC_SYNC();
            R.thr = 0.0; R.lp = 1.0; R.le = 0;
            if (role == 0) {
                BMPC_UNROLL
                for (int r = 0; r < NW; r++) {
                    const LDSD* cr = comb + (size_t)(r * 64 + lane) * TRIAL_COMB;
                    R.thr += cr[0]; R.lp *= cr[1]; R.le += (int)cr[2];
                }
                R.th = c[3]; R.f = c[4];
            }
        }
        if (live && role == 0) {
            GD P = A.part + pi;
            P[PT_F1 * A.NP] = R.f; P[PT_TH1 * A.NP] = R.th + R.thr;
            P[PT_LS1 * A.NP] = log(R.lp) + (double)R.le * 0.69314718055994530942;
        }
        const bool last = round >= A.o.trial_repeats;
        BMPC_FENCE_SYNC();
        if (live && role == 0 && k == 1 && (ls_instance(A, b, last) || last)) ended[li] = 1.0;
        BMPC_FENCE_SYNC();
        bool left = false;
        for (int q = 0; q < ipw; q++) left = left || (ended[q] == 0.0);
        if (!left) break;
    }
}
BMPC_KBODY void k_trial_body(const PipeArgs& A, int wave, int lane, LDSD* lds_par) { k_trial_body_t<1>(A, wave, lane, lds_par); }

constexpr int TRIAL_SPEC = 4;
static_assert(TRIAL_SPEC - 1 <= RIC_NATT - 1 && NSLOT + NZ <= KREC, "candidate trial points fit the speculative gain copies");
static_assert(TRIAL_SPEC * 64 * 3 + IPW_MAX <= TRIAL_SPEC * 64 * TRIAL_COMB, "k_trial_spec's LDS fits trial_lds_doubles(N, 4)");
BMPC_KBODY void k_trial_spec_body(const PipeArgs& A, int wave, int tid, LDSD* lds_par) {
    const int count = A.L.cnt[2], N = A.N;
    if (wave * ipw_of(N) >= count) return;
    const int lane = tid & 63, role = tid >> 6;
    const PairMap m = pair_map(A, A.L.trial, count, wave, lane);
    const int ipw = ipw_of(N), S = N - 1;
    (void)stage_params<true, 64 * TRIAL_SPEC>(A, A.L.trial, count, wave, tid, m, lds_par);
    LDSD* ended = lds_par + (size_t)ipw * NPARL;
    LDSD* comb = ended + IPW_MAX;
    LDSD* win = comb + TRIAL_SPEC * 64 * 3;
    if (tid < IPW_MAX) ended[tid] = (tid < ipw && wave * ipw + tid < count) ? 0.0 : 1.0;
    BMPC_SYNC();
    const int flip = A.st[m.b].flip;
    for (int round = 0;; round++) {
        int b = m.b, k = m.k, li = m.li;
        BMPC_OPAQUE_I(b); BMPC_OPAQUE_I(k); BMPC_OPAQUE_I(li);
        const size_t pi = pair_of(A, b, k);
        PGP pg = lds_par + li * NPARL;
        const bool live = m.valid && ended[li] == 0.0;
        const int bt0 = live ? A.st[b].bt : 0;
        const bool mine = live && bt0 + role <= 9;
        double alpha = live ? A.st[b].alpha : 0.0;
        for (int r = 0; r < role; r++) alpha *= 0.5;
        GD cand = A.kspec + ((size_t)b * (RIC_NATT - 1) + (size_t)(role > 0 ? role - 1 : 0)) * ((size_t)S * KREC);
        GD t_out = role > 0 ? cand + (size_t)(k - 1) - pi : nullptr;
        GD zeta_out = role > 0 ? cand + (size_t)NSLOT * S + (size_t)(k - 1) - pi : nullptr;
        TrialPart R;
        trial_part<WR_ALL>(A, pg, b, k, pi, mine, mine && role == 0 && round == 0, alpha, flip, R, t_out, zeta_out);
        {
            LDSD* c = comb + (size_t)(role * 64 + lane) * 3;
            c[0] = R.f; c[1] = R.th + R.thr; c[2] = log(R.lp) + (double)R.le * 0.69314718055994530942;
        }
        if (tid < IPW_MAX) win[tid] = -1.0;
        BMPC_FENCE_SYNC();
        if (live && role == 0 && k == 1) {
            for (int j = 0; j < TRIAL_SPEC && bt0 + j <= 9; j++) {
                double f1 = 0, th1 = 0, ls1 = 0;
                for (int kk = 0; kk < S; kk++) {
                    const LDSD* c = comb + (size_t)(j * 64 + lane + kk) * 3;
                    f1 += c[0]; th1 += c[1]; ls1 += c[2];
                }
                if (ls_decide(A, b, f1, th1, ls1, false)) { win[li] = (double)j; ended[li] = 1.0; break; }
            }
        }
        BMPC_FENCE_SYNC();
        if (m.valid) {
            const int w = (int)win[li];
            if (w > 0) {
                GCD src = A.kspec + ((size_t)b * (RIC_NATT - 1) + (size_t)(w - 1)) * ((size_t)S * KREC) + (size_t)(k - 1);
                GD to = oth_t(A, flip), zo = oth_zeta(A, flip);
                for (int f = role; f < NSLOT; f += TRIAL_SPEC) to[(size_t)f * A.NP + pi] = src[(size_t)f * S];
                for (int f = role; f < NZ; f += TRIAL_SPEC) zo[(size_t)f * A.NP + pi] = src[(size_t)(NSLOT + f) * S];
            }
        }
        bool left = false;
        for (int q = 0; q < ipw; q++) left = left || (ended[q] == 0.0);
        if (!left) break;
        BMPC_FENCE_SYNC();
    }
}

struct OutVisitor {
    double viol;
    GD gi;
    PGP pg; const SegCtx* C; const double* y; bool term;
    BMPC_INL void rowv(int s, double h, bool lower) {
        if (h > 1e-6) viol += h;
        if (gi) gi[s - S_EE] = lower ? -h : h;
    }
    BMPC_INL void skip(int s) {
        if (!gi || s < S_EE || s >= S_END || (s >= S_TSET && !term)) return;
        double v;
        if (s < S_ROTU) v = -pg[P_BSET + (s - S_EE) * 4 + C->s] - y[Z_PS];
        else if (s < S_PHI) { int c = (s - S_COL) / 15, rr = (s - S_COL) - 15 * c; v = -pg[P_BSETJ + rr * 6 + c] - C->sl[c]; }
        else v = -pg[P_BSET + (s - S_TSET) * 4 + C->n] - C->sl[5];
        gi[s - S_EE] = v;
    }
    BMPC_INL void diag(int, int, double, double) {}
    BMPC_INL void zdiag(int, int, double, double) {}
    BMPC_INL void pose(int s, const double*, int, double h) { rowv(s, h, (s >= S_ROTL && s < S_COL) || (s >= S_TROTL)); }
    template <int S0, int CNT> BMPC_INL void group(unsigned) {}
    template <int C_> BMPC_INL void point_begin(unsigned) {}
    template <int C_> BMPC_INL void point(int s, const double*, double h) { rowv(s, h, false); }
    template <int C_> BMPC_INL void point_end() {}
};

BMPC_KBODY void k_out_body(const PipeArgs& A, int wave, int lane, LDSD* lds_par) {
    const int count = A.L.cnt[8], N = A.N;
    if (wave * ipw_of(N) >= count) return;
    PairMap m = pair_map(A, A.L.done, count, wave, lane);
    PGP pg = stage_params(A, A.L.done, count, wave, lane, m, lds_par);
    if (!m.valid) return;
    const int k = m.k, n_w = 44 * N + 6;
    const size_t b = (size_t)A.src[m.b];
    const bool term = (k == N - 1);
    const size_t pi = m.pi;
    const DynC dc = make_dync(A.o.dt);
    GCD lbx = A.lbx + b * n_w;
    GCD ubx = A.ubx + b * n_w;
    double iw0[3];
    BMPC_UNROLL
    for (int c = 0; c < 3; c++) iw0[c] = lbx[28 * N + (3 + c) * N];
    StagePoint S;
    GCD zc = cur_zeta(A, A.st[m.b].flip);
    load_zeta(zc, A.NP, pi, S.zeta);
    stage_point(A, pg, iw0, k, dc, S);
    GD x = A.x + b * n_w;
    BMPC_UNROLL
    for (int j = 0; j < 7; j++) {
        x[j * N + k] = S.y[Z_Q + j]; x[7 * N + j * N + k] = S.y[Z_DQ + j];
        x[14 * N + j * N + k] = S.y[Z_DDQ + j]; x[21 * N + j * N + k] = S.y[Z_U + j];
    }
    BMPC_UNROLL
    for (int c = 0; c < 6; c++) { x[28 * N + c * N + k] = S.C.pose[c]; x[34 * N + c * N + k] = S.C.v[c]; }
    x[40 * N + 6 + k] = S.y[Z_RS]; x[41 * N + 6 + k] = S.y[Z_DRS];
    x[42 * N + 6 + k] = S.y[Z_PS]; x[43 * N + 6 + k] = S.y[Z_DPS];
    if (k == 1) {
        BMPC_UNROLL
        for (int blk = 0; blk < 4; blk++)
            BMPC_UNROLL
            for (int j = 0; j < 7; j++) x[blk * 7 * N + j * N] = lbx[blk * 7 * N + j * N];
        BMPC_UNROLL
        for (int c = 0; c < 6; c++) { x[28 * N + c * N] = lbx[28 * N + c * N]; x[34 * N + c * N] = lbx[34 * N + c * N]; }
        x[40 * N + 6] = S.zeta[Z_RS]; x[41 * N + 6] = 0.0; x[42 * N + 6] = S.zeta[Z_PS]; x[43 * N + 6] = 0.0;
    }
    if (term)
        BMPC_UNROLL
        for (int i = 0; i < 6; i++) x[40 * N + i] = S.y[Z_D + i];
    GD g = A.g ? A.g + b * (147 * (N - 1) + 21) : nullptr;
    OutVisitor V;
    V.viol = 0; V.gi = g ? g + 35 * (N - 1) + 112 * (k - 1) : nullptr; V.pg = pg; V.C = &S.C; V.y = S.y; V.term = term;
    walk_rows(pg, lbx, ubx, N, k, S.y, S.zeta, S.K, S.C, V);
    double rdef[NX];
    if (!term) {
        double zn[NX];
        BMPC_UNROLL
        for (int i = 0; i < NX; i++) zn[i] = zc[(size_t)i * A.NP + pi + 1];
        defect_all(S.zeta, zn, S.C.v + 3, dc, rdef);
        BMPC_UNROLL
        for (int i = 0; i < Z_D; i++) { double r = fabs(rdef[i]); if (r > 1e-6) V.viol += r; }
        if (g) {
            GD ge = g + 35 * k;
            BMPC_UNROLL
            for (int i = 0; i < 35; i++) ge[i] = 0.0;
            BMPC_UNROLL
            for (int i = 0; i < 21; i++) ge[i] = rdef[i];
            BMPC_UNROLL
            for (int a = 0; a < 3; a++) ge[24 + a] = rdef[Z_PI + a];
            ge[33] = rdef[Z_RS]; ge[34] = rdef[Z_PS];
        }
    }
    if (k == 1) {
        double x1fix[24];
        x1fix_eval(lbx, N, dc.dt, x1fix);
        BMPC_UNROLL
        for (int i = 0; i < 24; i++) { double r = fabs(x1fix[i] - S.zeta[i]); if (r > 1e-6) V.viol += r; }
        if (g) {
            BMPC_UNROLL
            for (int i = 0; i < 35; i++) g[i] = 0.0;
            BMPC_UNROLL
            for (int i = 0; i < 21; i++) g[i] = x1fix[i] - S.zeta[i];
            BMPC_UNROLL
            for (int a = 0; a < 3; a++) g[24 + a] = x1fix[Z_PI + a] - S.zeta[Z_PI + a];
        }
    }
    A.part[PT_F1 * A.NP + pi] = V.viol;
}

struct MultVisitor {
    const PipeArgs* A; size_t pi; int N, k;
    GCD zc;
    GD lg;
    GD lx;
    double bz[6], Fc[6][3], sPS, sRS, sD[6], lxq[7], lxdq[7], lxddq[7], znn[4], z1[2];
    BMPC_INL double zrow(int s) const { return zc[(size_t)s * A->NP + pi]; }
    BMPC_INL void skip(int s) {
        if (s >= S_EE && s < (k == N - 1 ? S_END : S_TSET)) lg[s - S_EE] = 0.0;
    }
    BMPC_INL void diag(int s, int pos, double coef, double) {
        const double z = zrow(s);
        if (s < S_NONNEG) {
            const int blk = s / 14, jj = (s / 2) % 7;
            lx[(size_t)blk * 7 * N + (size_t)jj * N + k] += coef * z;
            if (blk == 0) lxq[jj] += coef * z; else if (blk == 1) lxdq[jj] += coef * z; else if (blk == 2) lxddq[jj] += coef * z;
        } else if (s < S_RS1) {
            const int m = s - S_NONNEG;
            lx[(size_t)(40 + m) * N + 6 + k] = -z;
            znn[m] = z;
        } else lx[(size_t)40 * N + (s - S_D1)] = -z;
    }
    BMPC_INL void zdiag(int s, int, double, double) { z1[s - S_RS1] = zrow(s); }
    BMPC_INL void pose(int s, const double* a, int sel, double) {
        const double z = zrow(s);
        const bool lower = (s >= S_ROTL && s < S_COL) || (s >= S_TROTL);
        lg[s - S_EE] = lower ? -z : z;
        BMPC_UNROLL
        for (int c = 0; c < 6; c++) bz[c] += z * a[c];
        if (sel == 1) sPS -= z; else if (sel == 2) sRS -= z; else if (sel == 3) sD[5] -= z;
    }
    template <int S0, int CNT> BMPC_INL void group(unsigned) {}
    template <int C> BMPC_INL void point_begin(unsigned) {}
    template <int C> BMPC_INL void point(int s, const double* a, double) {
        const double z = zrow(s);
        lg[s - S_EE] = z;
        Fc[C][0] += z * a[0]; Fc[C][1] += z * a[1]; Fc[C][2] += z * a[2];
        sD[C] -= z;
    }
    template <int C> BMPC_INL void point_end() {}
};

template <int C>
BMPC_INL void point_forces_to_q(const KinT& K, const double Fc[6][3], double* cq) {
    if constexpr (C < 6) {
        constexpr int nj = PointNJ<C>::value;
        const double* pc = kin_point<C>(K);
        BMPC_UNROLL
        for (int i = 0; i < nj; i++) {
            double r[3] = {pc[0] - K.o[i][0], pc[1] - K.o[i][1], pc[2] - K.o[i][2]}, c[3];
            cross3r(K.zx[i], r, c);
            cq[i] += c[0] * Fc[C][0] + c[1] * Fc[C][1] + c[2] * Fc[C][2];
        }
        point_forces_to_q<C + 1>(K, Fc, cq);
    }
}

BMPC_KBODY void k_mult_body(const PipeArgs& A, int wave, int lane, LDSD* lds_par) {
    const int count = A.B, N = A.N;
    if (wave * ipw_of(N) >= count) return;
    PairMap m;
    {
        const int S_ = N - 1, ipw = ipw_of(N);
        int li = lane / S_, kk = lane - li * S_;
        int e = wave * ipw + li;
        m.valid = (li < ipw) && (e < count);
        if (!m.valid) { e = wave * ipw; kk = 0; li = 0; }
        m.b = e; m.k = kk + 1; m.li = li; m.pi = pair_of(A, m.b, m.k);
    }
    PGP pg = stage_params(A, (GCI)nullptr, count, wave, lane, m, lds_par);
    if (!m.valid) return;
    const int k = m.k, n_w = 44 * N + 6, n_g = 147 * (N - 1) + 21;
    const size_t b = (size_t)A.src[m.b];
    const bool term = (k == N - 1);
    const size_t pi = m.pi;
    const DynC dc = make_dync(A.o.dt);
    GCD lbx = A.lbx + b * n_w;
    GCD ubx = A.ubx + b * n_w;
    PGP wts = pg + P_W;
    double iw0[3];
    BMPC_UNROLL
    for (int c = 0; c < 3; c++) iw0[c] = lbx[28 * N + (3 + c) * N];
    StagePoint S;
    load_zeta(cur_zeta(A, A.st[m.b].flip), A.NP, pi, S.zeta);
    stage_point(A, pg, iw0, k, dc, S);
    double G[6][7], g12[12];
    kin_G(S.K, S.Jl, S.y + Z_DQ, G);
    cost_grad12(pg, S.C, term, g12);
    GD lx = A.lam_x + b * n_w;
    BMPC_UNROLL
    for (int f = 0; f < 40; f++) lx[(size_t)f * N + k] = 0.0;
    MultVisitor V;
    V.A = &A; V.pi = pi; V.N = N; V.k = k; V.zc = cur_z(A, A.st[m.b].flip);
    V.lg = A.lam_g + b * n_g + 35 * (N - 1) + 112 * (k - 1);
    V.lx = lx;
    V.sPS = 0; V.sRS = 0; V.z1[0] = 0; V.z1[1] = 0;
    BMPC_UNROLL
    for (int c = 0; c < 6; c++) { V.bz[c] = 0; V.sD[c] = 0; V.Fc[c][0] = 0; V.Fc[c][1] = 0; V.Fc[c][2] = 0; }
    BMPC_UNROLL
    for (int j = 0; j < 7; j++) { V.lxq[j] = 0; V.lxdq[j] = 0; V.lxddq[j] = 0; }
    BMPC_UNROLL
    for (int i = 0; i < 4; i++) V.znn[i] = 0;
    walk_rows(pg, lbx, ubx, N, k, S.y, S.zeta, S.K, S.C, V);
    double bz[6], bzv[6], fa[3];
    BMPC_UNROLL
    for (int c = 0; c < 6; c++) { bz[c] = V.bz[c] + g12[c]; bzv[c] = g12[6 + c]; }
    BMPC_UNROLL
    for (int a = 0; a < 3; a++) fa[a] = bzv[3 + a] + 0.5 * dc.dt * bz[3 + a];
    double cq[7], cdq[7];
    BMPC_UNROLL
    for (int j = 0; j < 7; j++) {
        double sq = V.lxq[j], sd = V.lxdq[j];
        BMPC_UNROLL
        for (int a = 0; a < 3; a++) {
            sq += S.Jl[a][j] * bz[a] + G[a][j] * bzv[a] + G[3 + a][j] * fa[a];
            sd += S.Jl[a][j] * bzv[a] + S.K.zx[j][a] * fa[a];
        }
        if (j >= 2 && j <= 4) sd += 2 * wts[6] * S.y[Z_DQ + j];
        cq[j] = sq; cdq[j] = sd;
    }
    point_forces_to_q<0>(S.K, V.Fc, cq);
    GD rec = A.hrec + hrec_of(A, m.b, m.k);
    BMPC_UNROLL
    for (int j = 0; j < 7; j++) { rec[M_CQ + j] = cq[j]; rec[M_CDQ + j] = cdq[j]; rec[M_CDDQ + j] = V.lxddq[j]; }
    BMPC_UNROLL
    for (int a = 0; a < 3; a++)
        BMPC_UNROLL
        for (int j = 0; j < 7; j++) { rec[M_GANG + 7 * a + j] = G[3 + a][j]; rec[M_ZX + 7 * a + j] = S.K.zx[j][a]; }
    BMPC_UNROLL
    for (int c = 0; c < 6; c++) { rec[M_BZ + c] = bz[c]; rec[M_BZV + c] = bzv[c]; }
    rec[M_GRS] = 2 * wts[9] * S.y[Z_RS] + V.sRS - V.znn[0];
    rec[M_GPS] = 2 * wts[9] * S.y[Z_PS] + V.sPS - V.znn[2];
    if (k == 1) {
        BMPC_UNROLL
        for (int f = 0; f < 40; f++) lx[(size_t)f * N] = 0.0;
        BMPC_UNROLL
        for (int f = 0; f < 4; f++) lx[(size_t)(40 + f) * N + 6] = 0.0;
    }
}

}
```

boundplanner_amd/csrc/bmpc_pipeline.hip:

```cpp
#include "bmpc_platform_hip.hpp"
#include <cstdlib>
#include <utility>

#define BMPC_NT 64
#include "bmpc_pair_kernels.hpp"
#include "bmpc_ric_kernel.hpp"
#include "bmpc_stage_matrix.hpp"
#include "bmpc_internal.hpp"

using namespace bmpc;

#ifndef BMPC_TRIAL_NW
#define BMPC_TRIAL_NW 1
#endif

#define DV(H) (*reinterpret_cast<const PipeArgs*>(&(H)))

__global__ __launch_bounds__(64) void bmpc_k_init_inst(PipeArgsH H) { k_init_inst_body(DV(H), blockIdx.x * 64 + threadIdx.x); }
extern __shared__ __attribute__((aligned(16))) double bmpc_dyn_lds[];
__global__ __launch_bounds__(64, 1) void bmpc_k_init(PipeArgsH H) { k_init_body(DV(H), blockIdx.x, threadIdx.x, (LDSD*)bmpc_dyn_lds); }
__global__ __launch_bounds__(64, 1) void bmpc_k_pose(PipeArgsH H) { k_pose_body(DV(H), blockIdx.x, threadIdx.x, (LDSD*)bmpc_dyn_lds); }
__global__ __launch_bounds__(64, 1) void bmpc_k_eval(PipeArgsH H) {
    k_eval_body<0>(DV(H), blockIdx.x, threadIdx.x, (LDSD*)bmpc_dyn_lds);
}
__global__ __launch_bounds__(64, 1) void bmpc_k_points(PipeArgsH H) { k_points_body(DV(H), blockIdx.x, threadIdx.x, (LDSD*)bmpc_dyn_lds); }
__global__ __launch_bounds__(64, 1) void bmpc_k_curv(PipeArgsH H) {
    __shared__ double lds[EM_DOUBLES + 8];
    k_curv_body(DV(H), blockIdx.x, threadIdx.x, (LDSD*)lds);
}
__global__ __launch_bounds__(64, 1) void bmpc_k_points_pose(PipeArgsH H, int nw) {
    if ((int)blockIdx.x < nw) k_points_body(DV(H), blockIdx.x, threadIdx.x, (LDSD*)bmpc_dyn_lds);
    else k_pose_body(DV(H), (int)blockIdx.x - nw, threadIdx.x, (LDSD*)bmpc_dyn_lds);
}
__global__ __launch_bounds__(64, 1) void bmpc_k_eval_curv(PipeArgsH H, int nw) {
    if ((int)blockIdx.x < nw) k_eval_body<0>(DV(H), blockIdx.x, threadIdx.x, (LDSD*)bmpc_dyn_lds);
    else k_curv_body(DV(H), (int)blockIdx.x - nw, threadIdx.x, (LDSD*)bmpc_dyn_lds);
}
__global__ __launch_bounds__(64, 1) void bmpc_k_eval_curv_split(PipeArgsH H, int nw) {
    if ((int)blockIdx.x < nw) k_eval_body<1>(DV(H), blockIdx.x, threadIdx.x, (LDSD*)bmpc_dyn_lds);
    else if ((int)blockIdx.x < 2 * nw) k_eval_body<2>(DV(H), (int)blockIdx.x - nw, threadIdx.x, (LDSD*)bmpc_dyn_lds);
    else k_curv_body(DV(H), (int)blockIdx.x - 2 * nw, threadIdx.x, (LDSD*)bmpc_dyn_lds);
}
__global__ __launch_bounds__(64, 1) void bmpc_k_eval_main(PipeArgsH H) { k_eval_body<1>(DV(H), blockIdx.x, threadIdx.x, (LDSD*)bmpc_dyn_lds); }
__global__ __launch_bounds__(64, 1) void bmpc_k_eval_chain(PipeArgsH H) { k_eval_body<2>(DV(H), blockIdx.x, threadIdx.x, (LDSD*)bmpc_dyn_lds); }
#ifndef BMPC_EVAL_SPLIT_WGS
#define BMPC_EVAL_SPLIT_WGS (1 << 30)
#endif
#ifndef BMPC_RIC_NT
#define BMPC_RIC_NT 128
#endif
#ifndef BMPC_RIC_SPEC_BELOW
#define BMPC_RIC_SPEC_BELOW 512
#endif
#ifndef BMPC_RIC_WPE
#define BMPC_RIC_WPE 3
#endif
__global__ __launch_bounds__(BMPC_RIC_NT, BMPC_RIC_WPE) __attribute__((disable_tail_calls)) void bmpc_k_ric(PipeArgsH H) {
    __shared__ __attribute__((aligned(16))) double lds[RIC_LDS_DOUBLES];
    k_ric_body<BMPC_RIC_NT, true>(ric_kernel_args(), blockIdx.x, threadIdx.x, (LDSD*)lds);
}
__global__ __launch_bounds__(BMPC_RIC_NT, 1) __attribute__((disable_tail_calls)) void bmpc_k_ric_lat(PipeArgsH H) {
    __shared__ __attribute__((aligned(16))) double lds[RIC_LDS_DOUBLES];
    k_ric_body<BMPC_RIC_NT, false>(ric_kernel_args(), blockIdx.x, threadIdx.x, (LDSD*)lds);
}
__global__ __launch_bounds__(BMPC_RIC_NT, 1) __attribute__((disable_tail_calls)) void bmpc_k_ric_att(PipeArgsH H) {
    __shared__ __attribute__((aligned(16))) double lds[RIC_LDS_DOUBLES];
    k_ric_att_body<BMPC_RIC_NT, false>(ric_kernel_args(), blockIdx.x, threadIdx.x, (LDSD*)lds);
}
__global__ __launch_bounds__(BMPC_RIC_NT, BMPC_RIC_WPE) __attribute__((disable_tail_calls)) void bmpc_k_ric_att_thr(PipeArgsH H) {
    __shared__ __attribute__((aligned(16))) double lds[RIC_LDS_DOUBLES];
    k_ric_att_body<BMPC_RIC_NT, true>(ric_kernel_args(), blockIdx.x, threadIdx.x, (LDSD*)lds);
}
__global__ __launch_bounds__(BMPC_RIC_NT, 1) __attribute__((disable_tail_calls)) void bmpc_k_ric_sel(PipeArgsH H) {
    __shared__ __attribute__((aligned(16))) double lds[RIC_LDS_DOUBLES];
    k_ric_body<BMPC_RIC_NT, false, true>(ric_kernel_args(), blockIdx.x, threadIdx.x, (LDSD*)lds);
}
#ifndef BMPC_RIC_LAT_BELOW
#define BMPC_RIC_LAT_BELOW 512
#endif
__global__ __launch_bounds__(64) void bmpc_k_fwd(PipeArgsH H) {
    __shared__ __attribute__((aligned(16))) double lds[FW_LDS_DOUBLES];
    k_fwd_body(DV(H), blockIdx.x, threadIdx.x, (LDSD*)lds);
}
__global__ __launch_bounds__(64, 1) void bmpc_k_step(PipeArgsH H) { k_step_body(DV(H), blockIdx.x, threadIdx.x, (LDSD*)bmpc_dyn_lds); }
__global__ __launch_bounds__(64) void bmpc_k_init_fin(PipeArgsH H) { k_init_fin_body(DV(H), blockIdx.x * 64 + threadIdx.x); }
__global__ __launch_bounds__(64) void bmpc_k_admit(PipeArgsH H) { k_admit_body(DV(H), blockIdx.x * 64 + threadIdx.x); }
__global__ void bmpc_k_pool_reset(PipeArgsH H, int done_too) { if (threadIdx.x == 0 && blockIdx.x == 0) k_pool_reset_body(DV(H), done_too != 0); }
__global__ __launch_bounds__(64 * BMPC_TRIAL_NW, BMPC_TRIAL_NW == 4 ? 2 : 1) void bmpc_k_trial(PipeArgsH H) {
    k_trial_body_t<BMPC_TRIAL_NW>(DV(H), blockIdx.x, threadIdx.x, (LDSD*)bmpc_dyn_lds);
}
__global__ __launch_bounds__(64 * TRIAL_SPEC, 1) void bmpc_k_trial_spec(PipeArgsH H) {
    k_trial_spec_body(DV(H), blockIdx.x, threadIdx.x, (LDSD*)bmpc_dyn_lds);
}
#ifndef BMPC_TRIAL_SPEC_WGS
#define BMPC_TRIAL_SPEC_WGS 256
#endif
__global__ void bmpc_k_rotate(PipeArgsH H) { if (threadIdx.x == 0 && blockIdx.x == 0) k_rotate_body(DV(H)); }
__global__ __launch_bounds__(64, 1) void bmpc_k_out(PipeArgsH H) { k_out_body(DV(H), blockIdx.x, threadIdx.x, (LDSD*)bmpc_dyn_lds); }
__global__ __launch_bounds__(64, 1) void bmpc_k_mult(PipeArgsH H) { k_mult_body(DV(H), blockIdx.x, threadIdx.x, (LDSD*)bmpc_dyn_lds); }
__global__ __launch_bounds__(64) void bmpc_k_mult_sweep(PipeArgsH H) { k_mult_sweep_body(DV(H), blockIdx.x * 64 + threadIdx.x); }
__global__ __launch_bounds__(64) void bmpc_k_fin(PipeArgsH H) { k_fin_body(DV(H), blockIdx.x * 64 + threadIdx.x); }

#define LAUNCH(kern, nb, nt)                                            \
    do {                                                                \
        if ((nb) > 0) hipLaunchKernelGGL(kern, dim3(nb), dim3(nt), 0, st, *A); \
    } while (0)
#define LAUNCH_DYN(kern, nb, nt, lds_doubles)                           \
    do {                                                                \
        if ((nb) > 0) hipLaunchKernelGGL(kern, dim3(nb), dim3(nt), (lds_doubles) * sizeof(double), st, *A); \
    } while (0)

extern "C" hipError_t bmpc_pipe_launch_init(const PipeArgsH* A, int n0, hipStream_t st) {
    LAUNCH(bmpc_k_init_inst, (n0 + 63) / 64, 64);
    LAUNCH_DYN(bmpc_k_init, waves_for(A->N, n0), 64, pair_lds_doubles(A->N, false));
    LAUNCH(bmpc_k_init_fin, (n0 + 63) / 64, 64);
    hipLaunchKernelGGL(bmpc_k_pool_reset, dim3(1), dim3(64), 0, st, *A, 0);
    return hipGetLastError();
}

extern "C" hipError_t bmpc_pipe_launch_retire_out(const PipeArgsH* A, int n_max, hipStream_t st) {
    LAUNCH_DYN(bmpc_k_out, waves_for(A->N, n_max), 64, pair_lds_doubles(A->N, false));
    LAUNCH(bmpc_k_fin, (n_max + 63) / 64, 64);
    return hipGetLastError();
}
extern "C" hipError_t bmpc_pipe_launch_retire_admit(const PipeArgsH* A, int n_max, int refill, hipStream_t st) {
    LAUNCH(bmpc_k_admit, (n_max + 63) / 64, 64);
    if (refill) {
        LAUNCH_DYN(bmpc_k_init, waves_for(A->N, n_max), 64, pair_lds_doubles(A->N, false));
        LAUNCH(bmpc_k_init_fin, (n_max + 63) / 64, 64);
    }
    hipLaunchKernelGGL(bmpc_k_pool_reset, dim3(1), dim3(64), 0, st, *A, 1);
    return hipGetLastError();
}

static void launch_eval(const PipeArgsH* A, int nw, hipStream_t st) {
    static const int split_launches = env_int("BMPC_SPLIT_LAUNCHES", 0);
    static const int eval_split_wgs = env_int("BMPC_EVAL_SPLIT_WGS", BMPC_EVAL_SPLIT_WGS);
    if (split_launches) {
        LAUNCH_DYN(bmpc_k_points, nw, 64, pair_lds_doubles(A->N, false));
        LAUNCH_DYN(bmpc_k_pose, nw, 64, pair_lds_doubles(A->N, false));
        if (nw <= eval_split_wgs) {
            LAUNCH_DYN(bmpc_k_eval_main, nw, 64, pair_lds_doubles(A->N, true));
            LAUNCH_DYN(bmpc_k_eval_chain, nw, 64, pair_lds_doubles(A->N, true));
        } else
            LAUNCH_DYN(bmpc_k_eval, nw, 64, pair_lds_doubles(A->N, true));
        LAUNCH(bmpc_k_curv, nw, 64);
    } else if (nw > 0) {
        hipLaunchKernelGGL(bmpc_k_points_pose, dim3(2 * nw), dim3(64), pair_lds_doubles(A->N, false) * sizeof(double), st, *A, nw);
        if (nw <= eval_split_wgs)
            hipLaunchKernelGGL(bmpc_k_eval_curv_split, dim3(A->o.hess == 2 ? 3 * nw : 2 * nw), dim3(64), pair_lds_doubles(A->N, true) * sizeof(double), st, *A, nw);
        else
            hipLaunchKernelGGL(bmpc_k_eval_curv, dim3(A->o.hess == 2 ? 2 * nw : nw), dim3(64), pair_lds_doubles(A->N, true) * sizeof(double), st, *A, nw);
    }
}

static void launch_direction(PipeArgsH* A, int n_act, int nw, hipStream_t st, hipEvent_t e0, hipEvent_t e1, int* was_lat) {
    static const int lat_below = env_int("BMPC_RIC_LAT_BELOW", BMPC_RIC_LAT_BELOW);
    if (e0) (void)hipEventRecord(e0, st);
    static const int spec_below = env_int("BMPC_RIC_SPEC_BELOW", BMPC_RIC_SPEC_BELOW);
    if (n_act < spec_below && n_act > 0) {
        const int natt = n_act * RIC_NATT <= 512 ? RIC_NATT : 1536 / n_act;
        A->natt = natt < 2 ? 2 : (natt > RIC_NATT ? RIC_NATT : natt);
        if (n_act * A->natt <= 512) LAUNCH(bmpc_k_ric_att, n_act * A->natt, BMPC_RIC_NT);
        else LAUNCH(bmpc_k_ric_att_thr, n_act * A->natt, BMPC_RIC_NT);
        LAUNCH(bmpc_k_ric_sel, n_act, BMPC_RIC_NT);
    } else if (n_act < lat_below) LAUNCH(bmpc_k_ric_lat, n_act, BMPC_RIC_NT);
    else LAUNCH(bmpc_k_ric, n_act, BMPC_RIC_NT);
    if (e1) (void)hipEventRecord(e1, st);
    if (was_lat) *was_lat = n_act < lat_below || n_act < spec_below;
    LAUNCH(bmpc_k_fwd, n_act, 64);
    LAUNCH_DYN(bmpc_k_step, nw, 64, pair_lds_doubles(A->N, false));
}

static void launch_trial(const PipeArgsH* A, int nw, hipStream_t st) {
    static const int trial_spec_wgs = env_int("BMPC_TRIAL_SPEC_WGS", BMPC_TRIAL_SPEC_WGS);
    if (nw <= trial_spec_wgs && A->NP == (size_t)(A->N - 1)) LAUNCH_DYN(bmpc_k_trial_spec, nw, 64 * TRIAL_SPEC, trial_lds_doubles(A->N, TRIAL_SPEC));
    else
        LAUNCH_DYN(bmpc_k_trial, nw, 64 * BMPC_TRIAL_NW, trial_lds_doubles(A->N, BMPC_TRIAL_NW));
}

static void swap_lists(PipeArgsH* A) { std::swap(A->L.eval, A->L.eval_next); std::swap(A->L.trial, A->L.trial_next); }
extern "C" hipError_t bmpc_pipe_launch_step(PipeArgsH* A, int n_act, hipStream_t st, hipEvent_t e0, hipEvent_t e1, int* was_lat) {
    const int nw = waves_for(A->N, n_act);
    launch_eval(A, nw, st);
    launch_direction(A, n_act, nw, st, e0, e1, was_lat);
    launch_trial(A, nw, st);
    LAUNCH(bmpc_k_rotate, 1, 64);
    swap_lists(A);
    return hipGetLastError();
}

extern "C" hipError_t bmpc_pipe_launch_mult(const PipeArgsH* A, hipStream_t st) {
    LAUNCH_DYN(bmpc_k_mult, waves_for(A->N, A->B), 64, pair_lds_doubles(A->N, false));
    LAUNCH(bmpc_k_mult_sweep, (A->B + 63) / 64, 64);
    return hipGetLastError();
}

__global__ __launch_bounds__(64) void bmpc_k_dbg_set_rows(PipeArgsH H, const double* t, const double* z, const int* mode) {
    k_set_rows_body(DV(H), (size_t)blockIdx.x * 64 + threadIdx.x, (GCD)t, (GCD)z, (GCI)mode);
}
__global__ __launch_bounds__(64) void bmpc_k_dbg_newton_out(PipeArgsH H, double* dzeta, double* dt, double* dz, double* state) {
    k_newton_out_body(DV(H), (size_t)blockIdx.x * 64 + threadIdx.x, (GD)dzeta, (GD)dt, (GD)dz, (GD)state);
}
__global__ __launch_bounds__(BMPC_RIC_NT, 1) void bmpc_k_dbg_stage_matrices(PipeArgsH H, const double* lam_pi, double* Hout) {
    __shared__ __attribute__((aligned(16))) double lds[RIC_LDS_DOUBLES];
    k_stage_matrix_body<BMPC_RIC_NT>(ric_kernel_args(), blockIdx.x, threadIdx.x, (LDSD*)lds, (GCD)lam_pi, (GD)Hout);
}
extern "C" hipError_t bmpc_pipe_launch_stage_matrices(const PipeArgsH* A, const double* d_t, const double* d_z, const double* d_lam_pi,
                                                      double* d_H, hipStream_t st) {
    const size_t nset = (size_t)A->B * (A->N - 1) * NSLOT;
    hipLaunchKernelGGL(bmpc_k_dbg_set_rows, dim3((unsigned)((nset + 63) / 64)), dim3(64), 0, st, *A, d_t, d_z, (const int*)nullptr);
    launch_eval(A, waves_for(A->N, A->B), st);
    hipLaunchKernelGGL(bmpc_k_dbg_stage_matrices, dim3(A->B), dim3(BMPC_RIC_NT), 0, st, *A, d_lam_pi, d_H);
    return hipGetLastError();
}

extern "C" hipError_t bmpc_pipe_launch_newton_step(PipeArgsH* A, const double* d_t, const double* d_z, const int* d_mode, double* d_dzeta,
                                                   double* d_dt, double* d_dz, double* d_state, hipStream_t st) {
    const size_t nset = (size_t)A->B * (A->N - 1) * NSLOT;
    const int nw = waves_for(A->N, A->B);
    hipLaunchKernelGGL(bmpc_k_dbg_set_rows, dim3((unsigned)((nset + 63) / 64)), dim3(64), 0, st, *A, d_t, d_z, d_mode);
    launch_eval(A, nw, st);
    launch_direction(A, A->B, nw, st, nullptr, nullptr, nullptr);
    hipLaunchKernelGGL(bmpc_k_dbg_newton_out, dim3((unsigned)((nset + 63) / 64)), dim3(64), 0, st, *A, d_dzeta, d_dt, d_dz, d_state);
    return hipGetLastError();
}

__global__ __launch_bounds__(64) void bmpc_k_dbg_ls_plant(PipeArgsH H, const double* plant, int after_step, int nan_other) {
    k_ls_plant_body(DV(H), (size_t)blockIdx.x * 64 + threadIdx.x, (GCD)plant, after_step, nan_other);
}
__global__ __launch_bounds__(64) void bmpc_k_dbg_ls_out(PipeArgsH H, double* zeta0, double* t0, double* z0, double* zeta1, double* t1,
                                                        double* z1, double* ls) {
    k_ls_out_body(DV(H), (size_t)blockIdx.x * 64 + threadIdx.x, (GD)zeta0, (GD)t0, (GD)z0, (GD)zeta1, (GD)t1, (GD)z1, (GD)ls);
}
__global__ __launch_bounds__(64) void bmpc_k_dbg_ctl_plant(PipeArgsH H, const double* plant) {
    k_ctl_plant_body(DV(H), (size_t)blockIdx.x * 64 + threadIdx.x, (GCD)plant);
}
__global__ __launch_bounds__(64) void bmpc_k_dbg_ctl_out(PipeArgsH H, double* ctl, int after_trial) {
    k_ctl_out_body(DV(H), (size_t)blockIdx.x * 64 + threadIdx.x, (GD)ctl, after_trial);
}
extern "C" hipError_t bmpc_pipe_launch_line_search(PipeArgsH* A, const double* d_t, const double* d_z, const int* d_mode,
                                                   const double* d_plant0, const double* d_plant1, double* d_dzeta, double* d_dt,
                                                   double* d_dz, double* d_state, double* d_zeta0, double* d_t0, double* d_z0,
                                                   double* d_zeta1, double* d_t1, double* d_z1, double* d_ls, hipStream_t st,
                                                   const double* d_ctl_plant, double* d_ctl) {
    const unsigned nbi = (unsigned)((A->B + 63) / 64);
    const size_t nset = (size_t)A->B * (A->N - 1) * NSLOT;
    const unsigned nb = (unsigned)((nset + 63) / 64);
    const int nw = waves_for(A->N, A->B);
    if (d_t) hipLaunchKernelGGL(bmpc_k_dbg_set_rows, dim3(nb), dim3(64), 0, st, *A, d_t, d_z, d_mode);
    if (d_t || d_plant0) hipLaunchKernelGGL(bmpc_k_dbg_ls_plant, dim3(nb), dim3(64), 0, st, *A, d_plant0, 0, d_t ? 1 : 0);
    if (d_ctl_plant) hipLaunchKernelGGL(bmpc_k_dbg_ctl_plant, dim3(nbi), dim3(64), 0, st, *A, d_ctl_plant);
    launch_eval(A, nw, st);
    launch_direction(A, A->B, nw, st, nullptr, nullptr, nullptr);
    hipLaunchKernelGGL(bmpc_k_dbg_newton_out, dim3(nb), dim3(64), 0, st, *A, d_dzeta, d_dt, d_dz, d_state);
    if (d_ctl) hipLaunchKernelGGL(bmpc_k_dbg_ctl_out, dim3(nbi), dim3(64), 0, st, *A, d_ctl, 0);
    if (d_plant1) hipLaunchKernelGGL(bmpc_k_dbg_ls_plant, dim3(nb), dim3(64), 0, st, *A, d_plant1, 1, 0);
    launch_trial(A, nw, st);
    hipLaunchKernelGGL(bmpc_k_dbg_ls_out, dim3(nb), dim3(64), 0, st, *A, d_zeta0, d_t0, d_z0, d_zeta1, d_t1, d_z1, d_ls);
    if (d_ctl) hipLaunchKernelGGL(bmpc_k_dbg_ctl_out, dim3(nbi), dim3(64), 0, st, *A, d_ctl, 1);
    return hipGetLastError();
}

extern "C" void bmpc_pipe_build_table(int* tbl) { build_scatter_table(tbl); }
extern "C" int bmpc_pipe_hrec(void) { return HREC; }
extern "C" int bmpc_pipe_krec(void) { return KREC; }
extern "C" int bmpc_pipe_npart(void) { return NPART; }
extern "C" void bmpc_pipe_ls_sizes(int* plant0, int* plant1, int* out) { *plant0 = LS_PLANT0; *plant1 = LS_PLANT1; *out = LS_OUT; }
extern "C" void bmpc_pipe_ctl_sizes(int* plant, int* out) { *plant = CTL_PLANT; *out = CTL_OUT; }
extern "C" size_t bmpc_pipe_state_bytes(void) { return sizeof(InstState); }
```

boundplanner_amd/csrc/bmpc_pipeline.hpp:

```cpp
#pragma once
#include "bmpc_stage.hpp"

namespace bmpc {

constexpr int F_CD = 0;
constexpr int F_P17 = F_CD + 35;
constexpr int F_H17 = F_P17 + 119;
constexpr int F_EW = F_H17 + 153;
constexpr int F_SUFZ = F_EW + 42;
constexpr int F_DGR = F_SUFZ + 21;
constexpr int F_DZ2 = F_DGR + 96;
constexpr int F_GZ2 = F_DZ2 + 2;
constexpr int F_RDEF = F_GZ2 + 6;
constexpr int F_MAIN_END = F_RDEF + 32;
constexpr int F_CQP = 512;
constexpr int F_CQQ = F_CQP + 21;
constexpr int F_CQD = F_CQQ + 49;
constexpr int F_END = F_CQD + 49;
constexpr int HREC = 640;
static_assert(F_MAIN_END <= F_CQP && F_CQP % 16 == 0 && F_END <= HREC && HREC % 64 == 0, "record layout");

BMPC_HD int dg_pos(int i) {
    if (i < 7) return Z_Q + i;
    if (i < 14) return Z_DQ + i - 7;
    if (i < 21) return Z_DDQ + i - 14;
    if (i < 28) return Z_U + i - 21;
    if (i == 28) return Z_RS;
    if (i == 29) return Z_DRS;
    if (i == 30) return Z_PS;
    if (i == 31) return Z_DPS;
    if (i < 38) return Z_D + i - 32;
    return Z_PI + i - 38;
}
constexpr int dg_pos_c(int i) {
    return i < 7 ? Z_Q + i : i < 14 ? Z_DQ + i - 7 : i < 21 ? Z_DDQ + i - 14 : i < 28 ? Z_U + i - 21 : i == 28 ? Z_RS
           : i == 29 ? Z_DRS : i == 30 ? Z_PS : i == 31 ? Z_DPS : i < 38 ? Z_D + i - 32 : Z_PI + i - 38;
}
BMPC_HD int pos17(int i) { return i < 7 ? Z_Q + i : (i < 14 ? Z_DQ + i - 7 : Z_PI + i - 14); }

constexpr int KREC = 320;
constexpr int RIC_NATT = 5 , RIC_FS_P0 = 24 * 25 / 2, RIC_FS_P = NPSYM - RIC_FS_P0, RIC_FS = 256;
static_assert(8 + RIC_FS_P + 16 <= RIC_FS, "forward-start record");
constexpr int NPART = 272;
constexpr int PT_FORCE = 16;
constexpr int PT_SIG = 169;
constexpr int PT_SIDE = 48, SD_CD = 0 , SD_CD5 = 35 , SD_HQQ = 42 , SD_GQ = 70 ,
              SD_DD = 91 , SD_GD = 97 , SD_KKT = 115 , SD_END = 121;
constexpr int PT_POSE = 184, PZ_M6 = 0 , PZ_MS = 21 , PZ_SS = 39 , PZ_BP0 = 42 , PZ_BP1 = 48, PZ_BPZ = 54,
              PZ_BS0 = 60 , PZ_BS1 = 63, PZ_BSZ = 66, PZ_BV = 69 , PZ_KKT = 75 , PZ_VANG = 81 , PZ_END = 84;
static_assert(PT_SIDE + SD_END <= PT_SIG && PT_SIG + 10 <= PT_POSE && PT_POSE + PZ_END <= NPART, "partials layout");
enum { PT_CMAX = 0, PT_CSUM, PT_CMIN, PT_ZSUM, PT_PRIM, PT_THETA, PT_LOGS, PT_NROWS, PT_FVAL,
       PT_AP, PT_AD, PT_DBAR, PT_DPHIF, PT_F1, PT_TH1, PT_LS1 };

constexpr int M_CQ = 0, M_CDQ = 7, M_CDDQ = 14, M_GANG = 21 , M_ZX = 42 , M_BZ = 63 , M_BZV = 69 ,
              M_GRS = 75, M_GPS = 76, M_END = 77;
static_assert(M_END <= HREC, "multiplier record fits the stage record");

enum { ST_EVAL = 0, ST_STEP = 1, ST_TRIAL = 2, ST_DONE = 3 };

struct InstState {
    int state, it, status, nfilt, hess_mode, bt, armijo, tries;
    int flip, stall;
    double mu, alpha, ad, ap, hreg, err_prev, filt_mu, theta_max, theta_min;
    int gn_skip, gn_back;
    int ksel, pad_;
    double dw_last, err_best;
    double f0, th0, ls0, D, phi0, fk;
    double filt_th[8], filt_phi[8];
};

template <int DEV> struct PtrT {
    typedef double* D; typedef const double* CD; typedef int* I; typedef const int* CI;
    typedef struct InstState* S; typedef const RobotConst* RC;
};
template <> struct PtrT<1> {
    typedef GD D; typedef GCD CD; typedef GI I; typedef GCI CI;
    typedef BMPC_AS1 struct InstState* S; typedef GRC RC;
};

template <int DEV> struct ListsT {
    typename PtrT<DEV>::I eval, step, trial, eval_next, trial_next;
    typename PtrT<DEV>::I curv;
    typename PtrT<DEV>::I done, admit;
    typename PtrT<DEV>::I cnt;
};
constexpr int NCNT = 14;

template <int DEV> struct PipeArgsT {
    typedef PtrT<DEV> PT;
    int B, N;
    int natt, pad0_;
    SolverOpts o;
    typename PT::RC rc;
    typename PT::CD x0, lbx, ubx, p;
    typename PT::D x, f, viol, g;
    typename PT::I iters, status;
    size_t NP, SS, HS, KS;
    typename PT::D zeta, zeta_t, dz;
    typename PT::D t, t_t, z, dt, z_t;
    typename PT::D hrec;
    typename PT::D krec;
    typename PT::D dx1;
    typename PT::D kspec, fspec;
    typename PT::D part;
    typename PT::S st;
    typename PT::I src;
    ListsT<DEV> L;
    typename PT::CI tbl;
    typename PT::D prof;
    typename PT::D lam_g, lam_x;
    typename PT::CI cont;
};
typedef PipeArgsT<0> PipeArgsH;
typedef PipeArgsT<1> PipeArgs;
static_assert(sizeof(PipeArgsH) == sizeof(PipeArgs), "host/device argument layouts differ");
typedef BMPC_AS1 InstState* GST;

template <class AT> BMPC_INL auto cur_t(const AT& A, int flip) -> decltype(A.t) { return flip ? A.t_t : A.t; }
template <class AT> BMPC_INL auto oth_t(const AT& A, int flip) -> decltype(A.t) { return flip ? A.t : A.t_t; }
template <class AT> BMPC_INL auto cur_z(const AT& A, int flip) -> decltype(A.z) { return flip ? A.z_t : A.z; }
template <class AT> BMPC_INL auto oth_z(const AT& A, int flip) -> decltype(A.z) { return flip ? A.z : A.z_t; }
template <class AT> BMPC_INL auto cur_zeta(const AT& A, int flip) -> decltype(A.zeta) { return flip ? A.zeta_t : A.zeta; }
template <class AT> BMPC_INL auto oth_zeta(const AT& A, int flip) -> decltype(A.zeta) { return flip ? A.zeta : A.zeta_t; }
template <class AT> BMPC_INL size_t pair_of(const AT& A, int b, int k) { return (size_t)b * A.SS + (k - 1); }
template <class AT> BMPC_INL size_t hrec_of(const AT& A, int b, int k) { return (size_t)b * A.HS + (size_t)(k - 1) * HREC; }
template <class AT> BMPC_INL size_t krec_of(const AT& A, int b, int k) { return (size_t)b * A.KS + (size_t)(k - 1) * KREC; }

constexpr size_t PIPE_SOA_FIELDS = 3 * (size_t)NZ + 5 * (size_t)NSLOT + NPART;
inline size_t pipe_slot_block(int N) { return ((PIPE_SOA_FIELDS + HREC + KREC) * (size_t)(N - 1) + 15) / 16 * 16 + 16; }
inline size_t pipe_np_field_major(int cap, int N) { return ((size_t)cap * (N - 1) + 63) / 64 * 64 + 64; }
inline size_t pipe_workspace_doubles(int cap, int N, int slot_major) {
    return (slot_major ? pipe_slot_block(N) * (size_t)cap + 64
                       : (PIPE_SOA_FIELDS + HREC + KREC) * pipe_np_field_major(cap, N)) + (size_t)cap * NX
           + (size_t)cap * ((size_t)(RIC_NATT - 1) * (N - 1) * KREC + (size_t)RIC_NATT * RIC_FS);
}
template <class AT> inline void pipe_carve(AT& A, double* w, int cap, int N, int slot_major) {
    const size_t S = (size_t)(N - 1);
    if (slot_major) { A.NP = S; A.SS = A.HS = A.KS = pipe_slot_block(N); }
    else { A.NP = pipe_np_field_major(cap, N); A.SS = S; A.HS = S * HREC; A.KS = S * KREC; }
    const size_t NP = A.NP;
    double* w0 = w;
    A.zeta = w; w += NZ * NP; A.zeta_t = w; w += NZ * NP; A.dz = w; w += NZ * NP;
    A.t = w; w += NSLOT * NP; A.t_t = w; w += NSLOT * NP; A.z = w; w += NSLOT * NP; A.dt = w; w += NSLOT * NP;
    A.z_t = w; w += NSLOT * NP;
    A.part = w; w += NPART * NP;
    if (slot_major) w = w0 + ((size_t)(w - w0) + 15) / 16 * 16;
    A.hrec = w; w += HREC * NP; A.krec = w; w += KREC * NP;
    A.dx1 = slot_major ? w0 + pipe_slot_block(N) * (size_t)cap + 64 : w;
    A.kspec = A.dx1 + (size_t)cap * NX;
    A.fspec = A.kspec + (size_t)cap * (RIC_NATT - 1) * (size_t)(N - 1) * KREC;
}

constexpr int EM_DOUBLES_C = 16 * 66 + 64;
constexpr int IPW_MAX = 8;
BMPC_HD int ipw_of(int N) { int i = 64 / (N - 1); return i < IPW_MAX ? i : IPW_MAX; }

struct PairMap { int b, k, li; bool valid; size_t pi; };
BMPC_INL PairMap pair_map(const PipeArgs& A, GCI list, int count, int wave, int lane) {
    const int S = A.N - 1, ipw = ipw_of(A.N);
    int li = lane / S, kk = lane - li * S;
    int e = wave * ipw + li;
    PairMap m;
    m.valid = (li < ipw) && (e < count);
    if (!m.valid) { e = wave * ipw; kk = 0; li = 0; }
    m.li = li;
    m.b = list[e]; m.k = kk + 1;
    m.pi = pair_of(A, m.b, m.k);
    return m;
}
BMPC_HD int waves_for(int N, int count) { int ipw = ipw_of(N); return (count + ipw - 1) / ipw; }

template <int NTHR = 64>
BMPC_INL void stage_masks(LDSD* lds_par, int ipw, int wave, int lane, int count) {
    for (int e = lane; e < ipw * 10; e += NTHR) {
        const int li = e / 10, c = e - 10 * li;
        if (wave * ipw + li < count) {
            PGP pg = lds_par + li * NPARL;
            unsigned mk = 0;
            for (int rr = 0; rr < 15; rr++) {
                PGP a = c < 6 ? pg + P_ASETJ + 45 * c : pg + P_ASET + 45 * (c - 6);
                const double bb = c < 6 ? pg[P_BSETJ + rr * 6 + c] + pg[P_SLACKS0 + c] : pg[P_BSET + rr * 4 + (c - 6)];
                if (!(a[rr] == 0 && a[rr + 15] == 0 && a[rr + 30] == 0 && bb > 0)) mk |= 1u << rr;
            }
            lds_par[li * NPARL + NPAR + c] = (double)mk;
        }
    }
    BMPC_SYNC();
}
template <bool BATCHED = true, int NTHR = 64>
BMPC_INL PGP stage_params(const PipeArgs& A, GCI list, int count, int wave, int lane, const PairMap& m, LDSD* lds_par) {
    const int ipw = ipw_of(A.N);
    if constexpr (!BATCHED) {
        for (int li = 0; li < ipw; li++) {
            const int e = wave * ipw + li;
            if (e < count) {
                GCD src = A.p + (size_t)A.src[list ? list[e] : e] * NPAR;
                for (int i = lane; i < NPAR; i += NTHR) lds_par[li * NPARL + i] = src[i];
            }
        }
        BMPC_SYNC();
        stage_masks<NTHR>(lds_par, ipw, wave, lane, count);
        return lds_par + m.li * NPARL;
    }
    constexpr int NJ = (NPAR + NTHR - 1) / NTHR;
    for (int l0 = 0; l0 < ipw; l0 += 3) {
        double v[3][NJ];
        BMPC_UNROLL
        for (int c = 0; c < 3; c++) {
            const int li = l0 + c, e = wave * ipw + li;
            const bool on = li < ipw && e < count;
            GCD src = A.p + (size_t)A.src[on ? (list ? list[e] : e) : (list ? list[wave * ipw] : wave * ipw)] * NPAR;
            BMPC_UNROLL
            for (int j = 0; j < NJ; j++) { const int i = lane + NTHR * j; v[c][j] = (i < NPAR) ? src[i] : 0.0; }
        }
        BMPC_UNROLL
        for (int c = 0; c < 3; c++) {
            const int li = l0 + c, e = wave * ipw + li;
            if (li < ipw && e < count)
                BMPC_UNROLL
                for (int j = 0; j < NJ; j++) { const int i = lane + NTHR * j; if (i < NPAR) lds_par[li * NPARL + i] = v[c][j]; }
        }
    }
    BMPC_SYNC();
    stage_masks<NTHR>(lds_par, ipw, wave, lane, count);
    return lds_par + m.li * NPARL;
}
constexpr int TRIAL_COMB = 5;
BMPC_HD size_t trial_lds_doubles(int N, int nw) { return (size_t)ipw_of(N) * NPARL + IPW_MAX + (nw > 1 ? (size_t)nw * 64 * TRIAL_COMB : 0); }
BMPC_HD size_t pair_lds_doubles(int N, bool with_tile) { return (size_t)ipw_of(N) * NPARL + (with_tile ? EM_DOUBLES_C + 8 : 0); }

constexpr int EM_LD = 66;
constexpr int EM_DOUBLES = 16 * EM_LD + 64;
static_assert(EM_DOUBLES == EM_DOUBLES_C, "emitter tile size");
template <bool HOLE> struct EmitterT {
    LDSD* tile;
    GD out;
    int lane, f;
    int h0, h1;
    BMPC_INL void init(LDSD* lds, GD out_, int lane_, size_t rec, bool valid, int f0 = 0, int hole0 = 0, int hole1 = 0) {
        tile = lds; out = out_; lane = lane_; f = f0;
        h0 = hole0; h1 = hole1;
        lds[16 * EM_LD + lane] = valid ? (double)rec : -1.0;
    }
    BMPC_INL void put(double v) {
        tile[(f & 15) * EM_LD + lane] = v;
        f++;
        if ((f & 15) == 0) flush();
    }
    BMPC_INL void flush() {
        BMPC_SYNC();
        const int ff = lane & 15, p0 = lane >> 4, c0 = f - 16;
        bool mine = true;
        if constexpr (HOLE) mine = (c0 + ff < h0) || (c0 + ff >= h1);
        BMPC_UNROLL
        for (int i = 0; i < 16; i++) {
            int pr = 4 * i + p0;
            double base = tile[16 * EM_LD + pr];
            double v = tile[ff * EM_LD + pr];
            if (base >= 0.0 && mine) out[(size_t)base + c0 + ff] = v;
        }
        BMPC_SYNC();
    }
    BMPC_INL void pad_to(int n) { while (f < n) put(0.0); }
};
typedef EmitterT<false> Emitter;
struct DirectEmitter {
    GD out; bool valid; int f;
    BMPC_INL void put(double v) { if (valid) out[f] = v; f++; }
};

}
```

Baseline: 123,500 solves/s.

## Add horizon-specialized pair kernels with compile-time N and strides

Adds separate translation units that compile the pair-stage kernels (points, pose, eval, step, trial) for fixed horizons N=20 and N=30. A PipeArgsN view makes N, NP and the slot strides compile-time constants, and SoA column/offset helpers fold the per-pair base into the pointer. The launcher dispatches to these specialized kernels when the layout is slot-major, and the build now compiles objects in parallel. The aim is cheaper address arithmetic and better unrolling and register allocation. In exchange it adds code duplication and larger binaries.

```diff
diff --git a/__graft_entry__.py b/__graft_entry__.py
--- a/__graft_entry__.py
+++ b/__graft_entry__.py
@@ -1,16 +1,20 @@
 import os
 import subprocess
 import sys
+from concurrent.futures import ThreadPoolExecutor
 
 ROOT = os.path.dirname(os.path.abspath(__file__))
 CSRC = os.path.join(ROOT, "boundplanner_amd", "csrc")
 HIP_LIB = os.path.join(CSRC, "libboundmpc_hip.so")
 _COMMON = ["bmpc_platform_hip.hpp", "bmpc_device.hpp", "bmpc_internal.hpp"]
 _HANDLE = ["bmpc_handle.hpp", "bmpc_pipeline.hpp", "bmpc_stage.hpp", "bmpc_robot.hpp", "../../include/boundmpc.h"]
+_PAIR = ["bmpc_pair_fixed.hpp", "bmpc_pipeline.hpp", "bmpc_pair_kernels.hpp", "bmpc_stage.hpp"]
 HIP_OBJS = {
     "bmpc_fk.o": ("bmpc_fk.hip", [], _COMMON),
     "bmpc_pipeline.o": ("bmpc_pipeline.hip", [], _COMMON + ["bmpc_pipeline.hpp", "bmpc_pair_kernels.hpp", "bmpc_ric_kernel.hpp",
                                                             "bmpc_stage.hpp", "bmpc_stage_matrix.hpp"]),
+    "bmpc_pair_n20.o": ("bmpc_pair_n20.hip", [], _COMMON + _PAIR),
+    "bmpc_pair_n30.o": ("bmpc_pair_n30.hip", [], _COMMON + _PAIR),
     "bmpc_loop.o": ("bmpc_loop.hip", [], _COMMON + ["bmpc_loop.hpp", "bmpc_freespace.hpp", "bmpc_robot.hpp", "../../include/boundmpc.h"]),
     "bmpc_capi.o": ("bmpc_capi.hip", [], _COMMON + _HANDLE + ["bmpc_staging.hpp"]),
     "bmpc_capi_batch.o": ("bmpc_capi_batch.hip", [], _COMMON + _HANDLE + ["bmpc_staging.hpp", "bmpc_ik.hpp", "bmpc_sets.hpp",
@@ -29,12 +33,14 @@
 
 def build():
     flags = ["--offload-arch=gfx950", "-O3", "-std=c++17", "-fPIC", "-ffp-contract=on"]
-    objs, relink = [], not os.path.exists(HIP_LIB)
+    objs, jobs, relink = [], [], not os.path.exists(HIP_LIB)
     for obj, (src, defs, hdrs) in HIP_OBJS.items():
         o = os.path.join(CSRC, obj)
         if _stale(o, [os.path.join(CSRC, f) for f in [src] + hdrs]):
-            subprocess.check_call(["hipcc", *flags, *defs, "-c", os.path.join(CSRC, src), "-o", o])
+            jobs.append(["hipcc", *flags, *defs, "-c", os.path.join(CSRC, src), "-o", o])
         objs.append(o)
+    with ThreadPoolExecutor(max_workers=max(1, min(int(os.environ.get("MAX_JOBS", "8")), 16))) as pool:
+        list(pool.map(subprocess.check_call, jobs))
     if relink or _stale(HIP_LIB, objs):
         subprocess.check_call(["hipcc", "--offload-arch=gfx950", "-shared", "-fPIC", "-o", HIP_LIB, *objs])
     subprocess.check_call(["make", "-C", os.path.join(ROOT, "oracle")], stdout=subprocess.DEVNULL)
diff --git a/boundplanner_amd/csrc/bmpc_internal.hpp b/boundplanner_amd/csrc/bmpc_internal.hpp
--- a/boundplanner_amd/csrc/bmpc_internal.hpp
+++ b/boundplanner_amd/csrc/bmpc_internal.hpp
@@ -44,7 +44,12 @@
                                         double* d_ctl = nullptr);
 void bmpc_pipe_ls_sizes(int* plant0, int* plant1, int* out);
 void bmpc_pipe_ctl_sizes(int* plant, int* out);
+long bmpc_pipe_fixed_launches(void);
 void bmpc_pipe_build_table(int* tbl);
+enum { FX_POINTS, FX_POSE, FX_EVAL_MAIN, FX_EVAL_CHAIN, FX_POINTS_POSE, FX_EVAL_CURV_SPLIT, FX_STEP, FX_TRIAL, FX_TRIAL_SPEC };
+typedef void (*bmpc_pair_launcher)(int kern, const bmpc::PipeArgsH* A, int nw, unsigned nb, unsigned nt, size_t lds_bytes, hipStream_t st);
+void bmpc_pair_launch_n20(int kern, const bmpc::PipeArgsH* A, int nw, unsigned nb, unsigned nt, size_t lds_bytes, hipStream_t st);
+void bmpc_pair_launch_n30(int kern, const bmpc::PipeArgsH* A, int nw, unsigned nb, unsigned nt, size_t lds_bytes, hipStream_t st);
 size_t bmpc_pipe_state_bytes(void);
 
 void bmpc_handle_retain(bmpc_handle* h);
diff --git a/boundplanner_amd/csrc/bmpc_pair_fixed.hpp b/boundplanner_amd/csrc/bmpc_pair_fixed.hpp
--- /dev/null
+++ b/boundplanner_amd/csrc/bmpc_pair_fixed.hpp
@@ -0,0 +1,55 @@
+#include "bmpc_platform_hip.hpp"
+
+#define BMPC_NT 64
+#include "bmpc_pair_kernels.hpp"
+#include "bmpc_internal.hpp"
+
+#ifndef BMPC_FIXED_N
+#error "BMPC_FIXED_N: the horizon this translation unit is compiled for"
+#endif
+
+using namespace bmpc;
+
+#define BMPC_CAT_(a, b) a##b
+#define BMPC_CAT(a, b) BMPC_CAT_(a, b)
+#define KN(stem) BMPC_CAT(BMPC_CAT(stem, _n), BMPC_FIXED_N)
+
+#define DVN(H) (*reinterpret_cast<const PipeArgsN<BMPC_FIXED_N>*>(&(H)))
+static_assert(sizeof(PipeArgsN<BMPC_FIXED_N>) == sizeof(PipeArgsH), "the fixed-horizon view adds nothing to the argument block");
+
+extern __shared__ __attribute__((aligned(16))) double bmpc_dyn_lds[];
+
+__global__ __launch_bounds__(64, 1) void KN(bmpc_k_points)(PipeArgsH H) { k_points_body(DVN(H), blockIdx.x, threadIdx.x, (LDSD*)bmpc_dyn_lds); }
+__global__ __launch_bounds__(64, 1) void KN(bmpc_k_pose)(PipeArgsH H) { k_pose_body(DVN(H), blockIdx.x, threadIdx.x, (LDSD*)bmpc_dyn_lds); }
+__global__ __launch_bounds__(64, 1) void KN(bmpc_k_eval_main)(PipeArgsH H) { k_eval_body<1>(DVN(H), blockIdx.x, threadIdx.x, (LDSD*)bmpc_dyn_lds); }
+__global__ __launch_bounds__(64, 1) void KN(bmpc_k_eval_chain)(PipeArgsH H) { k_eval_body<2>(DVN(H), blockIdx.x, threadIdx.x, (LDSD*)bmpc_dyn_lds); }
+__global__ __launch_bounds__(64, 1) void KN(bmpc_k_points_pose)(PipeArgsH H, int nw) {
+    if ((int)blockIdx.x < nw) k_points_body(DVN(H), blockIdx.x, threadIdx.x, (LDSD*)bmpc_dyn_lds);
+    else k_pose_body(DVN(H), (int)blockIdx.x - nw, threadIdx.x, (LDSD*)bmpc_dyn_lds);
+}
+__global__ __launch_bounds__(64, 1) void KN(bmpc_k_eval_curv_split)(PipeArgsH H, int nw) {
+    if ((int)blockIdx.x < nw) k_eval_body<1>(DVN(H), blockIdx.x, threadIdx.x, (LDSD*)bmpc_dyn_lds);
+    else if ((int)blockIdx.x < 2 * nw) k_eval_body<2>(DVN(H), (int)blockIdx.x - nw, threadIdx.x, (LDSD*)bmpc_dyn_lds);
+    else k_curv_body(DVN(H), (int)blockIdx.x - 2 * nw, threadIdx.x, (LDSD*)bmpc_dyn_lds);
+}
+__global__ __launch_bounds__(64, 1) void KN(bmpc_k_step)(PipeArgsH H) { k_step_body(DVN(H), blockIdx.x, threadIdx.x, (LDSD*)bmpc_dyn_lds); }
+__global__ __launch_bounds__(64, 1) void KN(bmpc_k_trial)(PipeArgsH H) { k_trial_body_t<1>(DVN(H), blockIdx.x, threadIdx.x, (LDSD*)bmpc_dyn_lds); }
+__global__ __launch_bounds__(64 * TRIAL_SPEC, 1) void KN(bmpc_k_trial_spec)(PipeArgsH H) {
+    k_trial_spec_body(DVN(H), blockIdx.x, threadIdx.x, (LDSD*)bmpc_dyn_lds);
+}
+
+extern "C" void KN(bmpc_pair_launch)(int kern, const PipeArgsH* A, int nw, unsigned nb, unsigned nt, size_t lds_bytes, hipStream_t st) {
+    if (nb == 0) return;
+    switch (kern) {
+    case FX_POINTS: hipLaunchKernelGGL(KN(bmpc_k_points), dim3(nb), dim3(nt), lds_bytes, st, *A); break;
+    case FX_POSE: hipLaunchKernelGGL(KN(bmpc_k_pose), dim3(nb), dim3(nt), lds_bytes, st, *A); break;
+    case FX_EVAL_MAIN: hipLaunchKernelGGL(KN(bmpc_k_eval_main), dim3(nb), dim3(nt), lds_bytes, st, *A); break;
+    case FX_EVAL_CHAIN: hipLaunchKernelGGL(KN(bmpc_k_eval_chain), dim3(nb), dim3(nt), lds_bytes, st, *A); break;
+    case FX_POINTS_POSE: hipLaunchKernelGGL(KN(bmpc_k_points_pose), dim3(nb), dim3(nt), lds_bytes, st, *A, nw); break;
+    case FX_EVAL_CURV_SPLIT: hipLaunchKernelGGL(KN(bmpc_k_eval_curv_split), dim3(nb), dim3(nt), lds_bytes, st, *A, nw); break;
+    case FX_STEP: hipLaunchKernelGGL(KN(bmpc_k_step), dim3(nb), dim3(nt), lds_bytes, st, *A); break;
+    case FX_TRIAL: hipLaunchKernelGGL(KN(bmpc_k_trial), dim3(nb), dim3(nt), lds_bytes, st, *A); break;
+    case FX_TRIAL_SPEC: hipLaunchKernelGGL(KN(bmpc_k_trial_spec), dim3(nb), dim3(nt), lds_bytes, st, *A); break;
+    default: abort();
+    }
+}
diff --git a/boundplanner_amd/csrc/bmpc_pair_kernels.hpp b/boundplanner_amd/csrc/bmpc_pair_kernels.hpp
--- a/boundplanner_amd/csrc/bmpc_pair_kernels.hpp
+++ b/boundplanner_amd/csrc/bmpc_pair_kernels.hpp
@@ -17,8 +17,14 @@
     BMPC_UNROLL
     for (int i = 0; i < NZ; i++) z[i] = arr[(size_t)i * NP + pi];
 }
-
-BMPC_INL void stage_point(const PipeArgs& A, PGP pg, const double* iw0, int k, const DynC dc, StagePoint& S) {
+template <class AT> BMPC_INL void load_zeta(const AT& A, GCD arr, size_t pi, double* z) {
+    GCD col = soa_col(A, arr, pi);
+    BMPC_UNROLL
+    for (int i = 0; i < NZ; i++) z[i] = col[soa_off(A, (size_t)i * A.NP, pi)];
+}
+
+template <class AT>
+BMPC_INL void stage_point(const AT& A, PGP pg, const double* iw0, int k, const DynC dc, StagePoint& S) {
     nat_all(S.zeta, dc, S.y);
     kin_chain(A.rc, S.y + Z_Q, S.K);
     kin_jlin(S.K, S.Jl);
@@ -162,18 +168,8 @@
     }
 }
 
-struct RowAcc {
-    const PipeArgs* A; size_t pi; bool valid; double ad;
-    GCD tc, zc;
+struct RowSums {
     double cmax, csum, cmin, zsum, prim, nrows;
-    BMPC_INL void init(const PipeArgs* A_, size_t pi_, bool valid_, double ad_, GCD tc_, GCD zc_) {
-        A = A_; pi = pi_; valid = valid_; ad = ad_; tc = tc_; zc = zc_;
-        cmax = 0; csum = 0; cmin = 1e300; zsum = 0; prim = 0; nrows = 0;
-    }
-    BMPC_INL void row(int s, double h, double& sg, double& r0, double& r1, double& zz) {
-        size_t o = (size_t)s * A->NP + pi;
-        row_tz(tc[o], zc[o], h, sg, r0, r1, zz);
-    }
     BMPC_INL void row_tz(double t, double z_in, double h, double& sg, double& r0, double& r1, double& zz) {
         zz = z_in;
         r1 = BMPC_RCP(t); sg = zz * r1; r0 = sg * (h + t);
@@ -183,13 +179,27 @@
         nrows += 1.0;
     }
 };
+template <class AT> struct RowAccT : RowSums {
+    const AT* A; size_t pi; bool valid; double ad;
+    GCD tc, zc;
+    BMPC_INL void init(const AT* A_, size_t pi_, bool valid_, double ad_, GCD tc_, GCD zc_) {
+        A = A_; pi = pi_; valid = valid_; ad = ad_; tc = tc_; zc = zc_;
+        cmax = 0; csum = 0; cmin = 1e300; zsum = 0; prim = 0; nrows = 0;
+    }
+    BMPC_INL void row(int s, double h, double& sg, double& r0, double& r1, double& zz) {
+        size_t o = (size_t)s * A->NP + pi;
+        row_tz(tc[o], zc[o], h, sg, r0, r1, zz);
+    }
+};
+typedef RowAccT<PipeArgs> RowAcc;
 
 template <int S0_, int CNT_> struct RowPre {
     static constexpr int S0 = S0_, CNT = CNT_;
     double t[CNT_], z[CNT_];
-    BMPC_INL void load(const PipeArgs& A, GCD tc, GCD zc, size_t pi) {
-        BMPC_UNROLL
-        for (int i = 0; i < CNT_; i++) { size_t o = (size_t)(S0_ + i) * A.NP + pi; t[i] = tc[o]; z[i] = zc[o]; }
+    template <class AT> BMPC_INL void load(const AT& A, GCD tc, GCD zc, size_t pi) {
+        GCD tb = soa_col(A, tc, pi), zb = soa_col(A, zc, pi);
+        BMPC_UNROLL
+        for (int i = 0; i < CNT_; i++) { size_t o = soa_off(A, (size_t)(S0_ + i) * A.NP, pi); t[i] = tb[o]; z[i] = zb[o]; }
     }
 };
 template <int I0_, int CNT_> struct BndPre {
@@ -205,8 +215,8 @@
     }
 };
 
-struct PointAsm {
-    RowAcc* R; const KinT* K;
+template <class AT> struct PointAsmT {
+    RowAccT<AT>* R; const KinT* K;
     double M3[6], mc[3], sc, b30[3], b31[3], b3z[3], bc0, bc1, bcz;
     double Hqq[28], gq0[7], gq1[7], gqz[7], dD[6], gD0[6], gD1[6], gDz[6], cd[6][7], Fc[6][3];
     double pt[15], pz[15];
@@ -218,10 +228,11 @@
     }
     BMPC_INL void skip(int) {}
     template <int C> BMPC_INL void point_begin(unsigned act) {
+        GCD tb = soa_col(*R->A, R->tc, R->pi), zb = soa_col(*R->A, R->zc, R->pi);
         BMPC_UNROLL
         for (int i = 0; i < 15; i++) {
-            size_t o = (size_t)(S_COL + 15 * C + i) * R->A->NP + R->pi;
-            if ((act >> i) & 1u) { pt[i] = R->tc[o]; pz[i] = R->zc[o]; } else { pt[i] = 1.0; pz[i] = 0.0; }
+            size_t o = soa_off(*R->A, (size_t)(S_COL + 15 * C + i) * R->A->NP, R->pi);
+            if ((act >> i) & 1u) { pt[i] = tb[o]; pz[i] = zb[o]; } else { pt[i] = 1.0; pz[i] = 0.0; }
         }
         BMPC_UNROLL
         for (int i = 0; i < 6; i++) M3[i] = 0;
@@ -269,6 +280,7 @@
         for (int a = 0; a < 3; a++) Fc[C][a] = b3z[a];
     }
 };
+typedef PointAsmT<PipeArgs> PointAsm;
 
 struct PointRes {
     GCD base; size_t NP;
@@ -298,7 +310,7 @@
 };
 
 struct PoseAsm {
-    RowAcc* R;
+    RowSums* R;
     double M6[21], mS[3][6], sS[3], bp0[6], bp1[6], bpz[6], bS0[3], bS1[3], bSz[3];
     BMPC_INL void init(const double* Hp, const double* g12) {
         BMPC_UNROLL
@@ -406,7 +418,7 @@
 }
 
 struct DiagAsm {
-    RowAcc* R;
+    RowSums* R;
     double D, g0, g1, gz;
     BMPC_INL void begin() { D = 0; g0 = 0; g1 = 0; gz = 0; }
     BMPC_INL void diag(double coef, double h, double t, double z) {
@@ -468,9 +480,9 @@
         chain_all<J + 1>(K, Jl, G, hdt, M6, Hv, PR, E);
     }
 }
-template <int I, int IEND, class RP, class BP, class EM>
-BMPC_INL void p17_emit_all(const PipeArgs& A, PGP pg, const RP& rp, const BP& bp, int k, const double* y, const KinT& K,
-                           const double Jl[3][7], const double G[6][7], double hdt, RowAcc& R, const PointRes& PA,
+template <int I, int IEND, class AT, class RP, class BP, class EM>
+BMPC_INL void p17_emit_all(const AT& A, PGP pg, const RP& rp, const BP& bp, int k, const double* y, const KinT& K,
+                           const double Jl[3][7], const double G[6][7], double hdt, RowSums& R, const PointRes& PA,
                            const PoseAsm& P, const double* bv, EM& E) {
     if constexpr (I < IEND) {
         PGP wts = pg + P_W;
@@ -576,9 +588,9 @@
         }
 }
 
-template <int I, class RP, class BP, class EM>
-BMPC_INL void dg_emit_all(const PipeArgs& A, PGP pg, const RP& rp, const BP& bp, int k, bool term,
-                          const double* y, RowAcc& R, const PointRes& PA, const PoseAsm& PO, EM& E) {
+template <int I, class AT, class RP, class BP, class EM>
+BMPC_INL void dg_emit_all(const AT& A, PGP pg, const RP& rp, const BP& bp, int k, bool term,
+                          const double* y, RowSums& R, const PointRes& PA, const PoseAsm& PO, EM& E) {
     if constexpr (I < 38) {
         PGP wts = pg + P_W;
         DiagAsm dgv;
@@ -615,7 +627,8 @@
     }
 }
 
-BMPC_KBODY void k_pose_body(const PipeArgs& A, int wave, int lane, LDSD* lds_par) {
+template <class AT>
+BMPC_KBODY void k_pose_body(const AT& A, int wave, int lane, LDSD* lds_par) {
     const int count = A.L.cnt[0], N = A.N;
     if (wave * ipw_of(N) >= count) return;
     PairMap m = pair_map(A, A.L.eval, count, wave, lane);
@@ -630,7 +643,7 @@
     StagePoint S;
     const int flip = A.st[m.b].flip;
     GCD zc = cur_zeta(A, flip), tc = cur_t(A, flip), zcur = cur_z(A, flip);
-    load_zeta(zc, A.NP, m.pi, S.zeta);
+    load_zeta(A, zc, m.pi, S.zeta);
     RowPre<S_EE, 21> rp_pose;
     rp_pose.load(A, tc, zcur, m.pi);
     const double t_phi = tc[(size_t)S_PHI * A.NP + m.pi], z_phi = zcur[(size_t)S_PHI * A.NP + m.pi];
@@ -662,7 +675,7 @@
             Sg[(size_t)(4 + bb) * A.NP] = c2 * ge;
         }
     }
-    RowAcc R;
+    RowAccT<AT> R;
     R.init(&A, m.pi, m.valid, 0.0, tc, zcur);
     PoseAsm PO;
     PO.R = &R;
@@ -703,8 +716,8 @@
     for (int a = 0; a < 3; a++) Pz[(size_t)(PZ_VANG + a) * A.NP] = S.C.v[3 + a];
 }
 
-template <int MODE>
-BMPC_KBODY void k_eval_body(const PipeArgs& A, int wave, int lane, LDSD* lds) {
+template <int MODE, class AT>
+BMPC_KBODY void k_eval_body(const AT& A, int wave, int lane, LDSD* lds) {
     const int count = A.L.cnt[0], N = A.N;
     if (wave * ipw_of(N) >= count) return;
     PairMap m = pair_map(A, A.L.eval, count, wave, lane);
@@ -717,7 +730,7 @@
     if constexpr (MODE == 2) {
         struct { double zeta[NZ], y[NZ]; KinT K; double Jl[3][7]; } S;
         const int flip = A.st[m.b].flip;
-        load_zeta(cur_zeta(A, flip), A.NP, m.pi, S.zeta);
+        load_zeta(A, cur_zeta(A, flip), m.pi, S.zeta);
         nat_all(S.zeta, dc, S.y);
         kin_chain(A.rc, S.y + Z_Q, S.K);
         kin_jlin(S.K, S.Jl);
@@ -743,13 +756,13 @@
     struct { double zeta[NZ], y[NZ]; KinT K; double Jl[3][7]; } S;
     const int flip = A.st[m.b].flip;
     GCD zc = cur_zeta(A, flip), tc = cur_t(A, flip), zcur = cur_z(A, flip);
-    load_zeta(zc, A.NP, m.pi, S.zeta);
+    load_zeta(A, zc, m.pi, S.zeta);
     nat_all(S.zeta, dc, S.y);
     kin_chain(A.rc, S.y + Z_Q, S.K);
     kin_jlin(S.K, S.Jl);
     double G[6][7];
     kin_G(S.K, S.Jl, S.y + Z_DQ, G);
-    RowAcc R;
+    RowAccT<AT> R;
     R.init(&A, m.pi, m.valid, ad, tc, zcur);
     PoseAsm PO;
     PO.R = &R;
@@ -836,7 +849,7 @@
             for (int a = 0; a < 3; a++) E.put(mm < 7 ? sufz[mm < 7 ? mm : 0][a] : 0.0);
     }
     double zeta2[NZ], y2[NZ];
-    load_zeta(zc, A.NP, m.pi, zeta2);
+    load_zeta(A, zc, m.pi, zeta2);
     nat_all(zeta2, dc, y2);
     RowPre<28, 40> rp_b;
     BndPre<14, 14> bp_b;
@@ -896,7 +909,8 @@
     }
 }
 
-BMPC_KBODY void k_points_body(const PipeArgs& A, int wave, int lane, LDSD* lds_par) {
+template <class AT>
+BMPC_KBODY void k_points_body(const AT& A, int wave, int lane, LDSD* lds_par) {
     const int count = A.L.cnt[0], N = A.N;
     if (wave * ipw_of(N) >= count) return;
     PairMap m = pair_map(A, A.L.eval, count, wave, lane);
@@ -908,19 +922,19 @@
     PGP pg = stage_params(A, A.L.eval, count, wave, lane, m, lds_par);
     double zeta[NZ], y[NZ];
     const int flip = A.st[m.b].flip;
-    load_zeta(cur_zeta(A, flip), A.NP, m.pi, zeta);
+    load_zeta(A, cur_zeta(A, flip), m.pi, zeta);
     nat_all(zeta, dc, y);
     KinT K;
     kin_chain(A.rc, y + Z_Q, K);
     SegCtx C;
     BMPC_UNROLL
     for (int i = 0; i < 6; i++) C.sl[i] = pg[P_SLACKS0 + i] + y[Z_D + i];
-    RowAcc R;
+    RowAccT<AT> R;
     R.init(&A, m.pi, m.valid, 0.0, cur_t(A, flip), cur_z(A, flip));
-    PointAsm PA;
+    PointAsmT<AT> PA;
     PA.R = &R; PA.K = &K;
     PA.init();
-    walk_points<PointAsm, 0>(pg, K, C.sl, PA);
+    walk_points<PointAsmT<AT>, 0>(pg, K, C.sl, PA);
     if (!m.valid) return;
     GD Sd = A.part + (size_t)PT_SIDE * A.NP + m.pi;
     BMPC_UNROLL
@@ -950,7 +964,8 @@
     }
 }
 
-BMPC_KBODY void k_curv_body(const PipeArgs& A, int wave, int lane, LDSD* lds) {
+template <class AT>
+BMPC_KBODY void k_curv_body(const AT& A, int wave, int lane, LDSD* lds) {
     const int count = A.L.cnt[10], N = A.N;
     if (A.o.hess != 2 || wave * ipw_of(N) >= count) return;
     PairMap m = pair_map(A, A.L.curv, count, wave, lane);
@@ -959,7 +974,7 @@
     E.init(lds, A.hrec, lane, hrec_of(A, m.b, m.k), m.valid, F_CQP);
     BMPC_SYNC();
     double zeta[NZ], y[NZ];
-    load_zeta(cur_zeta(A, A.st[m.b].flip), A.NP, m.pi, zeta);
+    load_zeta(A, cur_zeta(A, A.st[m.b].flip), m.pi, zeta);
     nat_all(zeta, dc, y);
     KinT K;
     double Jl[3][7];
@@ -1003,7 +1018,8 @@
     E.pad_to(HREC);
 }
 
-BMPC_INL void ls0_instance(const PipeArgs& A, int b) {
+template <class AT>
+BMPC_INL void ls0_instance(const AT& A, int b) {
     const int N = A.N;
     GST st = A.st + b;
     GCD P = A.part + pair_of(A, b, 1);
@@ -1065,15 +1081,16 @@
     }
     return false;
 }
-BMPC_INL bool ls_instance(const PipeArgs& A, int b, bool requeue) {
+template <class AT>
+BMPC_INL bool ls_instance(const AT& A, int b, bool requeue) {
     GCD P = A.part + pair_of(A, b, 1);
     double f1 = 0, th1 = 0, ls1 = 0;
     for (int k = 0; k < A.N - 1; k++) { f1 += P[PT_F1 * A.NP + k]; th1 += P[PT_TH1 * A.NP + k]; ls1 += P[PT_LS1 * A.NP + k]; }
     return ls_decide(A, b, f1, th1, ls1, requeue);
 }
 
-struct StepVisitor {
-    const PipeArgs* A; size_t pi; bool valid;
+template <class AT> struct StepVisitorT {
+    const AT* A; size_t pi; bool valid;
     double mu, tau;
     const double* dy;
     const double* dzt;
@@ -1083,16 +1100,17 @@
     double rp, rdn, rdd, dbar;
     template <int S0, int CNT> BMPC_INL void group(unsigned act) {
         static_assert(CNT <= ROW_GROUP_MAX, "row group size");
+        GCD tb = soa_col(*A, tc, pi), zb = soa_col(*A, zc, pi);
         BMPC_UNROLL
         for (int i = 0; i < CNT; i++) {
-            size_t o = (size_t)(S0 + i) * A->NP + pi;
-            if ((act >> i) & 1u) { gt[i] = tc[o]; gz[i] = zc[o]; } else { gt[i] = 1.0; gz[i] = 0.0; }
+            size_t o = soa_off(*A, (size_t)(S0 + i) * A->NP, pi);
+            if ((act >> i) & 1u) { gt[i] = tb[o]; gz[i] = zb[o]; } else { gt[i] = 1.0; gz[i] = 0.0; }
         }
     }
     BMPC_INL void fin(int s, double h, double adot) {
         const double c = -h - adot, t = gt[s - row_group_base(s)], z = gz[s - row_group_base(s)];
         const double rt = BMPC_RCP(t), dti = c - t, dzi = (mu - z * c) * rt;
-        if (valid) { size_t o = (size_t)s * A->NP + pi; A->dt[o] = c; }
+        if (valid) { size_t o = soa_off(*A, (size_t)s * A->NP, pi); soa_col(*A, A->dt, pi)[o] = c; }
         rp = fmax(rp, -dti * rt);
         if (-dzi * rdd > rdn * z) { rdn = -dzi; rdd = z; }
         dbar -= mu * dti * rt;
@@ -1115,6 +1133,7 @@
     }
     template <int C> BMPC_INL void point_end() {}
 };
+typedef StepVisitorT<PipeArgs> StepVisitor;
 
 template <int C>
 BMPC_INL void point_dirs(const KinT& K, const double* dyq, double dpt[6][3]) {
@@ -1133,7 +1152,8 @@
     }
 }
 
-BMPC_KBODY void k_step_body(const PipeArgs& A, int wave, int lane, LDSD* lds_par) {
+template <class AT>
+BMPC_KBODY void k_step_body(const AT& A, int wave, int lane, LDSD* lds_par) {
     const int count = A.L.cnt[1], N = A.N;
     if (wave * ipw_of(N) >= count) return;
     PairMap m = pair_map(A, A.L.step, count, wave, lane);
@@ -1150,15 +1170,15 @@
     for (int c = 0; c < 3; c++) iw0[c] = lbx[28 * N + (3 + c) * N];
     StagePoint S;
     const int flip = A.st[m.b].flip;
-    load_zeta(cur_zeta(A, flip), A.NP, m.pi, S.zeta);
+    load_zeta(A, cur_zeta(A, flip), m.pi, S.zeta);
     double dzt[NZ], dy[NZ];
-    load_zeta(A.dz, A.NP, m.pi, dzt);
+    load_zeta(A, A.dz, m.pi, dzt);
     nat_all(S.zeta, dc, S.y);
     nat_all(dzt, dc, dy);
-    StepVisitor V;
+    StepVisitorT<AT> V;
     V.A = &A; V.pi = m.pi; V.valid = m.valid; V.mu = mu; V.tau = fmax(0.99, 1.0 - mu); V.tc = cur_t(A, flip); V.zc = cur_z(A, flip);
     V.dy = dy; V.dzt = dzt; V.rp = 0.0; V.rdn = 0.0; V.rdd = 1.0; V.dbar = 0.0;
-    walk_rows<StepVisitor, WR_BOX>(pg, lbx, ubx, N, k, S.y, S.zeta, S.K, S.C, V);
+    walk_rows<StepVisitorT<AT>, WR_BOX>(pg, lbx, ubx, N, k, S.y, S.zeta, S.K, S.C, V);
     BMPC_PIN(V.rp); BMPC_PIN(V.rdn); BMPC_PIN(V.rdd); BMPC_PIN(V.dbar);
     BMPC_UNROLL
     for (int j = 0; j < 7; j++) BMPC_PIN(S.y[Z_Q + j]);
@@ -1212,9 +1232,9 @@
             double gg = 2 * wts[10] * S.y[Z_D + i] + (i != 4 ? 2 * wts[8] * (pg[P_SLACKS0 + i] + S.y[Z_D + i]) : 0.0);
             dphi_f += gg * dy[Z_D + i];
         }
-    walk_rows<StepVisitor, WR_POSE>(pg, lbx, ubx, N, k, S.y, S.zeta, S.K, S.C, V);
+    walk_rows<StepVisitorT<AT>, WR_POSE>(pg, lbx, ubx, N, k, S.y, S.zeta, S.K, S.C, V);
     BMPC_PIN(V.rp); BMPC_PIN(V.rdn); BMPC_PIN(V.rdd); BMPC_PIN(V.dbar);
-    walk_rows<StepVisitor, WR_PT0 | WR_PT1>(pg, lbx, ubx, N, k, S.y, S.zeta, S.K, S.C, V);
+    walk_rows<StepVisitorT<AT>, WR_PT0 | WR_PT1>(pg, lbx, ubx, N, k, S.y, S.zeta, S.K, S.C, V);
     if (m.valid) {
         GD P = A.part + m.pi;
         P[PT_DPHIF * A.NP] = dphi_f;
@@ -1224,8 +1244,8 @@
     if (m.valid && m.k == 1) ls0_instance(A, m.b);
 }
 
-struct TrialVisitor {
-    const PipeArgs* A; size_t pi; bool valid;
+template <class AT> struct TrialVisitorT {
+    const AT* A; size_t pi; bool valid;
     double alpha;
     GCD tc; GD tn_out;
     bool dual; double ad, mu; GCD zc; GD zn_out;
@@ -1235,15 +1255,17 @@
     template <int S0, int CNT> BMPC_INL void group(unsigned act) {
         static_assert(CNT <= ROW_GROUP_MAX, "row group size");
         double gz[CNT];
+        GCD tb = soa_col(*A, tc, pi), cb = soa_col(*A, A->dt, pi), zb = soa_col(*A, zc, pi);
         BMPC_UNROLL
         for (int i = 0; i < CNT; i++) {
-            size_t o = (size_t)(S0 + i) * A->NP + pi;
-            if ((act >> i) & 1u) { gt[i] = tc[o]; gc[i] = A->dt[o]; gz[i] = zc[o]; } else { gt[i] = 1.0; gc[i] = 1.0; gz[i] = 0.0; }
+            size_t o = soa_off(*A, (size_t)(S0 + i) * A->NP, pi);
+            if ((act >> i) & 1u) { gt[i] = tb[o]; gc[i] = cb[o]; gz[i] = zb[o]; } else { gt[i] = 1.0; gc[i] = 1.0; gz[i] = 0.0; }
         }
         if (dual) {
+            GD zo = soa_col(*A, zn_out, pi);
             BMPC_UNROLL
             for (int i = 0; i < CNT; i++)
-                if (gz[i] > 0.0) zn_out[(size_t)(S0 + i) * A->NP + pi] = gz[i] + ad * ((mu - gz[i] * gc[i]) * BMPC_RCP(gt[i]));
+                if (gz[i] > 0.0) zo[soa_off(*A, (size_t)(S0 + i) * A->NP, pi)] = gz[i] + ad * ((mu - gz[i] * gc[i]) * BMPC_RCP(gt[i]));
         }
     }
     BMPC_INL void fin(int s, double h) {
@@ -1253,7 +1275,7 @@
         thr += fabs(h + tn);
         int e;
         lp = frexp(lp * tn, &e); le += e;
-        if (valid) tn_out[(size_t)s * A->NP + pi] = tn;
+        if (valid) soa_col(*A, tn_out, pi)[soa_off(*A, (size_t)s * A->NP, pi)] = tn;
     }
     BMPC_INL void skip(int) {}
     BMPC_INL void diag(int s, int, double, double h) { fin(s, h); }
@@ -1263,10 +1285,11 @@
     template <int C> BMPC_INL void point(int s, const double*, double h) { fin(s, h); }
     template <int C> BMPC_INL void point_end() {}
 };
+typedef TrialVisitorT<PipeArgs> TrialVisitor;
 
 struct TrialPart { double f, th, thr, lp; int le; };
-template <int ROLES>
-BMPC_INL void trial_part(const PipeArgs& A, PGP pg, int b, int k, size_t pi, bool live, bool dual, double alpha, int flip, TrialPart& R,
+template <int ROLES, class AT>
+BMPC_INL void trial_part(const AT& A, PGP pg, int b, int k, size_t pi, bool live, bool dual, double alpha, int flip, TrialPart& R,
                          GD t_out = nullptr, GD zeta_out = nullptr) {
     const int N = A.N, n_w = 44 * N + 6;
     const bool term = (k == N - 1);
@@ -1284,10 +1307,10 @@
             for (int i = 0; i < NZ; i++) zo[(size_t)i * A.NP + pi] = S.zeta[i];
     }
     nat_all(S.zeta, dc, S.y);
-    TrialVisitor V;
+    TrialVisitorT<AT> V;
     V.A = &A; V.pi = pi; V.valid = live; V.alpha = alpha; V.thr = 0.0; V.lp = 1.0; V.le = 0; V.tc = cur_t(A, flip); V.tn_out = t_out ? t_out : oth_t(A, flip);
     V.dual = dual; V.ad = A.st[b].ad; V.mu = A.st[b].mu; V.zc = cur_z(A, flip); V.zn_out = oth_z(A, flip);
-    if constexpr ((ROLES & WR_BOX) != 0) walk_rows<TrialVisitor, WR_BOX>(pg, lbx, ubx, N, k, S.y, S.zeta, S.K, S.C, V);
+    if constexpr ((ROLES & WR_BOX) != 0) walk_rows<TrialVisitorT<AT>, WR_BOX>(pg, lbx, ubx, N, k, S.y, S.zeta, S.K, S.C, V);
     BMPC_SCHED_FENCE();
     if constexpr ((ROLES & (WR_POSE | WR_PT0 | WR_PT1)) != 0) kin_chain(A.rc, S.y + Z_Q, S.K);
     R.th = 0.0; R.f = 0.0;
@@ -1316,16 +1339,16 @@
         BMPC_UNROLL
         for (int a = 0; a < 3; a++) { S.C.pose[a] = S.K.pee[a]; S.C.pose[3 + a] = S.y[Z_PI + a] + 0.5 * dc.dt * S.C.v[3 + a]; }
         seg_ctx_eval(pg, A.N, k, S.y, iw0, S.C);
-        walk_rows<TrialVisitor, WR_POSE>(pg, lbx, ubx, N, k, S.y, S.zeta, S.K, S.C, V);
+        walk_rows<TrialVisitorT<AT>, WR_POSE>(pg, lbx, ubx, N, k, S.y, S.zeta, S.K, S.C, V);
         R.th = th; R.f = S.C.fv;
     }
     BMPC_SCHED_FENCE();
-    if constexpr ((ROLES & (WR_PT0 | WR_PT1)) != 0) walk_rows<TrialVisitor, ROLES & (WR_PT0 | WR_PT1)>(pg, lbx, ubx, N, k, S.y, S.zeta, S.K, S.C, V);
+    if constexpr ((ROLES & (WR_PT0 | WR_PT1)) != 0) walk_rows<TrialVisitorT<AT>, ROLES & (WR_PT0 | WR_PT1)>(pg, lbx, ubx, N, k, S.y, S.zeta, S.K, S.C, V);
     R.thr = V.thr; R.lp = V.lp; R.le = V.le;
 }
 
-template <int NW>
-BMPC_KBODY void k_trial_body_t(const PipeArgs& A, int wave, int tid, LDSD* lds_par) {
+template <int NW, class AT>
+BMPC_KBODY void k_trial_body_t(const AT& A, int wave, int tid, LDSD* lds_par) {
     static_assert(NW == 1 || NW == 4, "parts of the trial walk");
     const int count = A.L.cnt[2], N = A.N;
     if (wave * ipw_of(N) >= count) return;
@@ -1386,7 +1409,8 @@
 constexpr int TRIAL_SPEC = 4;
 static_assert(TRIAL_SPEC - 1 <= RIC_NATT - 1 && NSLOT + NZ <= KREC, "candidate trial points fit the speculative gain copies");
 static_assert(TRIAL_SPEC * 64 * 3 + IPW_MAX <= TRIAL_SPEC * 64 * TRIAL_COMB, "k_trial_spec's LDS fits trial_lds_doubles(N, 4)");
-BMPC_KBODY void k_trial_spec_body(const PipeArgs& A, int wave, int tid, LDSD* lds_par) {
+template <class AT>
+BMPC_KBODY void k_trial_spec_body(const AT& A, int wave, int tid, LDSD* lds_par) {
     const int count = A.L.cnt[2], N = A.N;
     if (wave * ipw_of(N) >= count) return;
     const int lane = tid & 63, role = tid >> 6;
@@ -1490,7 +1514,7 @@
     for (int c = 0; c < 3; c++) iw0[c] = lbx[28 * N + (3 + c) * N];
     StagePoint S;
     GCD zc = cur_zeta(A, A.st[m.b].flip);
-    load_zeta(zc, A.NP, pi, S.zeta);
+    load_zeta(A, zc, pi, S.zeta);
     stage_point(A, pg, iw0, k, dc, S);
     GD x = A.x + b * n_w;
     BMPC_UNROLL
@@ -1637,7 +1661,7 @@
     BMPC_UNROLL
     for (int c = 0; c < 3; c++) iw0[c] = lbx[28 * N + (3 + c) * N];
     StagePoint S;
-    load_zeta(cur_zeta(A, A.st[m.b].flip), A.NP, pi, S.zeta);
+    load_zeta(A, cur_zeta(A, A.st[m.b].flip), pi, S.zeta);
     stage_point(A, pg, iw0, k, dc, S);
     double G[6][7], g12[12];
     kin_G(S.K, S.Jl, S.y + Z_DQ, G);
diff --git a/boundplanner_amd/csrc/bmpc_pair_n20.hip b/boundplanner_amd/csrc/bmpc_pair_n20.hip
--- /dev/null
+++ b/boundplanner_amd/csrc/bmpc_pair_n20.hip
@@ -0,0 +1,2 @@
+#define BMPC_FIXED_N 20
+#include "bmpc_pair_fixed.hpp"
diff --git a/boundplanner_amd/csrc/bmpc_pair_n30.hip b/boundplanner_amd/csrc/bmpc_pair_n30.hip
--- /dev/null
+++ b/boundplanner_amd/csrc/bmpc_pair_n30.hip
@@ -0,0 +1,2 @@
+#define BMPC_FIXED_N 30
+#include "bmpc_pair_fixed.hpp"
diff --git a/boundplanner_amd/csrc/bmpc_pipeline.hip b/boundplanner_amd/csrc/bmpc_pipeline.hip
--- a/boundplanner_amd/csrc/bmpc_pipeline.hip
+++ b/boundplanner_amd/csrc/bmpc_pipeline.hip
@@ -1,4 +1,5 @@
 #include "bmpc_platform_hip.hpp"
+#include <atomic>
 #include <cstdlib>
 #include <utility>
 
@@ -133,21 +134,43 @@
     return hipGetLastError();
 }
 
+static bmpc_pair_launcher fixed_launcher(const PipeArgsH* A) {
+    static const int fixed_stride = env_int("BMPC_FIXED_STRIDE", 1);
+    if (!fixed_stride || A->NP != (size_t)(A->N - 1)) return nullptr;
+    return A->N == 20 ? bmpc_pair_launch_n20 : A->N == 30 ? bmpc_pair_launch_n30 : nullptr;
+}
+static std::atomic<long> fixed_launches{0};
+extern "C" long bmpc_pipe_fixed_launches(void) { return fixed_launches.load(); }
+#define LAUNCH_FX(fx, kern, nb, nt, lds_doubles) \
+    (fixed_launches++, fx(kern, A, nw, (unsigned)(nb), (unsigned)(nt), (lds_doubles) * sizeof(double), st))
+
 static void launch_eval(const PipeArgsH* A, int nw, hipStream_t st) {
     static const int split_launches = env_int("BMPC_SPLIT_LAUNCHES", 0);
     static const int eval_split_wgs = env_int("BMPC_EVAL_SPLIT_WGS", BMPC_EVAL_SPLIT_WGS);
+    const bmpc_pair_launcher fx = fixed_launcher(A);
     if (split_launches) {
-        LAUNCH_DYN(bmpc_k_points, nw, 64, pair_lds_doubles(A->N, false));
-        LAUNCH_DYN(bmpc_k_pose, nw, 64, pair_lds_doubles(A->N, false));
-        if (nw <= eval_split_wgs) {
+        if (fx) {
+            LAUNCH_FX(fx, FX_POINTS, nw, 64, pair_lds_doubles(A->N, false));
+            LAUNCH_FX(fx, FX_POSE, nw, 64, pair_lds_doubles(A->N, false));
+        } else {
+            LAUNCH_DYN(bmpc_k_points, nw, 64, pair_lds_doubles(A->N, false));
+            LAUNCH_DYN(bmpc_k_pose, nw, 64, pair_lds_doubles(A->N, false));
+        }
+        if (nw <= eval_split_wgs && fx) {
+            LAUNCH_FX(fx, FX_EVAL_MAIN, nw, 64, pair_lds_doubles(A->N, true));
+            LAUNCH_FX(fx, FX_EVAL_CHAIN, nw, 64, pair_lds_doubles(A->N, true));
+        } else if (nw <= eval_split_wgs) {
             LAUNCH_DYN(bmpc_k_eval_main, nw, 64, pair_lds_doubles(A->N, true));
             LAUNCH_DYN(bmpc_k_eval_chain, nw, 64, pair_lds_doubles(A->N, true));
         } else
             LAUNCH_DYN(bmpc_k_eval, nw, 64, pair_lds_doubles(A->N, true));
         LAUNCH(bmpc_k_curv, nw, 64);
     } else if (nw > 0) {
-        hipLaunchKernelGGL(bmpc_k_points_pose, dim3(2 * nw), dim3(64), pair_lds_doubles(A->N, false) * sizeof(double), st, *A, nw);
-        if (nw <= eval_split_wgs)
+        if (fx) LAUNCH_FX(fx, FX_POINTS_POSE, 2 * nw, 64, pair_lds_doubles(A->N, false));
+        else hipLaunchKernelGGL(bmpc_k_points_pose, dim3(2 * nw), dim3(64), pair_lds_doubles(A->N, false) * sizeof(double), st, *A, nw);
+        if (nw <= eval_split_wgs && fx)
+            LAUNCH_FX(fx, FX_EVAL_CURV_SPLIT, A->o.hess == 2 ? 3 * nw : 2 * nw, 64, pair_lds_doubles(A->N, true));
+        else if (nw <= eval_split_wgs)
             hipLaunchKernelGGL(bmpc_k_eval_curv_split, dim3(A->o.hess == 2 ? 3 * nw : 2 * nw), dim3(64), pair_lds_doubles(A->N, true) * sizeof(double), st, *A, nw);
         else
             hipLaunchKernelGGL(bmpc_k_eval_curv, dim3(A->o.hess == 2 ? 2 * nw : nw), dim3(64), pair_lds_doubles(A->N, true) * sizeof(double), st, *A, nw);
@@ -169,12 +192,18 @@
     if (e1) (void)hipEventRecord(e1, st);
     if (was_lat) *was_lat = n_act < lat_below || n_act < spec_below;
     LAUNCH(bmpc_k_fwd, n_act, 64);
-    LAUNCH_DYN(bmpc_k_step, nw, 64, pair_lds_doubles(A->N, false));
+    if (const bmpc_pair_launcher fx = fixed_launcher(A)) LAUNCH_FX(fx, FX_STEP, nw, 64, pair_lds_doubles(A->N, false));
+    else LAUNCH_DYN(bmpc_k_step, nw, 64, pair_lds_doubles(A->N, false));
 }
 
 static void launch_trial(const PipeArgsH* A, int nw, hipStream_t st) {
     static const int trial_spec_wgs = env_int("BMPC_TRIAL_SPEC_WGS", BMPC_TRIAL_SPEC_WGS);
-    if (nw <= trial_spec_wgs && A->NP == (size_t)(A->N - 1)) LAUNCH_DYN(bmpc_k_trial_spec, nw, 64 * TRIAL_SPEC, trial_lds_doubles(A->N, TRIAL_SPEC));
+    const bmpc_pair_launcher fx = fixed_launcher(A);
+    if (nw <= trial_spec_wgs && A->NP == (size_t)(A->N - 1)) {
+        if (fx) LAUNCH_FX(fx, FX_TRIAL_SPEC, nw, 64 * TRIAL_SPEC, trial_lds_doubles(A->N, TRIAL_SPEC));
+        else LAUNCH_DYN(bmpc_k_trial_spec, nw, 64 * TRIAL_SPEC, trial_lds_doubles(A->N, TRIAL_SPEC));
+    } else if (fx && BMPC_TRIAL_NW == 1)
+        LAUNCH_FX(fx, FX_TRIAL, nw, 64, trial_lds_doubles(A->N, 1));
     else
         LAUNCH_DYN(bmpc_k_trial, nw, 64 * BMPC_TRIAL_NW, trial_lds_doubles(A->N, BMPC_TRIAL_NW));
 }
diff --git a/boundplanner_amd/csrc/bmpc_pipeline.hpp b/boundplanner_amd/csrc/bmpc_pipeline.hpp
--- a/boundplanner_amd/csrc/bmpc_pipeline.hpp
+++ b/boundplanner_amd/csrc/bmpc_pipeline.hpp
@@ -116,6 +116,18 @@
 static_assert(sizeof(PipeArgsH) == sizeof(PipeArgs), "host/device argument layouts differ");
 typedef BMPC_AS1 InstState* GST;
 
+template <int NF> struct PipeArgsN;
+template <class AT> struct FixedView { static constexpr bool value = false; };
+template <int NF> struct FixedView<PipeArgsN<NF>> { static constexpr bool value = true; };
+template <class AT, class P> BMPC_INL P soa_col(const AT&, P arr, size_t pi) {
+    if constexpr (FixedView<AT>::value) return arr + pi;
+    else return arr;
+}
+template <class AT> BMPC_INL size_t soa_off(const AT&, size_t off, size_t pi) {
+    if constexpr (FixedView<AT>::value) return off;
+    else return off + pi;
+}
+
 template <class AT> BMPC_INL auto cur_t(const AT& A, int flip) -> decltype(A.t) { return flip ? A.t_t : A.t; }
 template <class AT> BMPC_INL auto oth_t(const AT& A, int flip) -> decltype(A.t) { return flip ? A.t : A.t_t; }
 template <class AT> BMPC_INL auto cur_z(const AT& A, int flip) -> decltype(A.z) { return flip ? A.z_t : A.z; }
@@ -127,7 +139,13 @@
 template <class AT> BMPC_INL size_t krec_of(const AT& A, int b, int k) { return (size_t)b * A.KS + (size_t)(k - 1) * KREC; }
 
 constexpr size_t PIPE_SOA_FIELDS = 3 * (size_t)NZ + 5 * (size_t)NSLOT + NPART;
-inline size_t pipe_slot_block(int N) { return ((PIPE_SOA_FIELDS + HREC + KREC) * (size_t)(N - 1) + 15) / 16 * 16 + 16; }
+constexpr size_t pipe_slot_block(int N) { return ((PIPE_SOA_FIELDS + HREC + KREC) * (size_t)(N - 1) + 15) / 16 * 16 + 16; }
+template <int NF> struct PipeArgsN : PipeArgs {
+    static_assert(NF >= 3, "horizon");
+    static constexpr int N = NF;
+    static constexpr size_t NP = (size_t)(NF - 1);
+    static constexpr size_t SS = pipe_slot_block(NF), HS = SS, KS = SS;
+};
 inline size_t pipe_np_field_major(int cap, int N) { return ((size_t)cap * (N - 1) + 63) / 64 * 64 + 64; }
 inline size_t pipe_workspace_doubles(int cap, int N, int slot_major) {
     return (slot_major ? pipe_slot_block(N) * (size_t)cap + 64
@@ -156,7 +174,7 @@
 BMPC_HD int ipw_of(int N) { int i = 64 / (N - 1); return i < IPW_MAX ? i : IPW_MAX; }
 
 struct PairMap { int b, k, li; bool valid; size_t pi; };
-BMPC_INL PairMap pair_map(const PipeArgs& A, GCI list, int count, int wave, int lane) {
+template <class AT> BMPC_INL PairMap pair_map(const AT& A, GCI list, int count, int wave, int lane) {
     const int S = A.N - 1, ipw = ipw_of(A.N);
     int li = lane / S, kk = lane - li * S;
     int e = wave * ipw + li;
@@ -187,8 +205,8 @@
     }
     BMPC_SYNC();
 }
-template <bool BATCHED = true, int NTHR = 64>
-BMPC_INL PGP stage_params(const PipeArgs& A, GCI list, int count, int wave, int lane, const PairMap& m, LDSD* lds_par) {
+template <bool BATCHED = true, int NTHR = 64, class AT>
+BMPC_INL PGP stage_params(const AT& A, GCI list, int count, int wave, int lane, const PairMap& m, LDSD* lds_par) {
     const int ipw = ipw_of(A.N);
     if constexpr (!BATCHED) {
         for (int li = 0; li < ipw; li++) {
```

New measurement: 128,700 solves/s (median of 6 runs). 1.04x the previous value.
